# SYSTRAN/faster-whisper

Measured on AMD Instinct MI355X. Metric: audio-sec/sec (RTF) large-v3 fp16 beam=5 batch=16, higher is better.
Workload: dtype f16

## Files before the change

faster_whisper_amd/_lib.py:

```python
import ctypes as C
import os

import numpy as np

_HERE = os.path.dirname(os.path.abspath(__file__))
LIB_PATH = os.environ.get("FWAMD_LIB") or os.path.join(_HERE, "libfwamd.so")

FW_OK = 0
FW_EINVAL = -1
FW_ENODEV = -2
FW_ENOMEM = -3
FW_ERUNTIME = -4
FW_ENOSPC = -5

COMPUTE_FLOAT16 = 0
COMPUTE_INT8_FLOAT16 = 1
FW_DT_F32 = 0
FW_DT_F16 = 1
FW_MAX_ALIGN_HEADS = 64


class FwConfig(C.Structure):
    _fields_ = [
        ("n_mels", C.c_int32), ("n_audio_ctx", C.c_int32), ("d_model", C.c_int32), ("n_heads", C.c_int32),
        ("n_enc_layers", C.c_int32), ("n_dec_layers", C.c_int32), ("n_vocab", C.c_int32),
        ("n_text_ctx", C.c_int32), ("is_multilingual", C.c_int32),
        ("tok_eot", C.c_int32), ("tok_sot", C.c_int32), ("tok_lang_begin", C.c_int32), ("n_langs", C.c_int32),
        ("tok_translate", C.c_int32), ("tok_transcribe", C.c_int32), ("tok_sot_lm", C.c_int32),
        ("tok_sot_prev", C.c_int32), ("tok_no_speech", C.c_int32), ("tok_no_timestamps", C.c_int32),
        ("tok_timestamp_begin", C.c_int32),
        ("n_suppress_begin", C.c_int32), ("suppress_begin", C.c_int32 * 8),
        ("n_align_heads", C.c_int32), ("align_heads", C.c_int32 * (2 * FW_MAX_ALIGN_HEADS)),
    ]


class FwWeight(C.Structure):
    _fields_ = [("name", C.c_char_p), ("data", C.c_void_p), ("dtype", C.c_int32), ("ndim", C.c_int32),
                ("dims", C.c_int64 * 4)]


class FwGenOpts(C.Structure):
    _fields_ = [
        ("beam_size", C.c_int32), ("patience", C.c_float), ("num_hypotheses", C.c_int32),
        ("length_penalty", C.c_float), ("repetition_penalty", C.c_float), ("no_repeat_ngram_size", C.c_int32),
        ("max_length", C.c_int32), ("return_scores", C.c_int32), ("return_no_speech_prob", C.c_int32),
        ("max_initial_timestamp_index", C.c_int32), ("suppress_blank", C.c_int32),
        ("suppress_tokens", C.POINTER(C.c_int32)), ("n_suppress_tokens", C.c_int32),
        ("sampling_topk", C.c_int32), ("sampling_temperature", C.c_float), ("seed", C.c_uint64),
        ("min_new_tokens", C.c_int32),
    ]


class FwVadWeights(C.Structure):
    _fields_ = [
        ("stft_basis", C.c_void_p), ("conv_w", C.c_void_p * 4), ("conv_b", C.c_void_p * 4),
        ("lstm_w", C.c_void_p), ("lstm_r", C.c_void_p), ("lstm_b", C.c_void_p), ("dec_w", C.c_void_p),
        ("dec_b", C.c_float),
    ]


SYMBOLS = [
    "fw_last_error", "fw_abi_version", "fw_device_count",
    "fw_model_create", "fw_model_free", "fw_model_info", "fw_model_blob", "fw_model_create_from_blob_dev",
    "fw_model_set_decode_batch", "fw_model_decode_batch", "fw_model_join_decoder", "fw_model_decode_stats",
    "fw_model_set_merge_wait", "fw_model_set_decode_lanes", "fw_model_run_capacity", "fw_dec_big_min_rows", "fw_dec_big_min_rows_of", "fw_test_knob",
    "fw_test_idle_lead_chunks",
    "fw_pack_blob_size", "fw_pack_blob_copy", "fw_pack_blob_free",
    "fw_logmel", "fw_logmel_full",
    "fw_encode", "fw_encode_pcm", "fw_encode_pcm_dev", "fw_tensor_shape", "fw_tensor_to_host",
    "fw_tensor_from_host", "fw_tensor_free",
    "fw_generate", "fw_detect_language", "fw_align",
    "fw_prof_enable", "fw_prof_reset", "fw_prof_count", "fw_prof_name", "fw_prof_get", "fw_synchronize",
    "fw_dev_alloc", "fw_dev_free", "fw_dev_upload",
    "fw_test_gemm", "fw_test_layernorm", "fw_test_attention", "fw_test_dec_linear", "fw_test_dec_logits", "fw_test_logits_rules",
    "fw_test_dec_self_attn", "fw_test_dec_cross_attn", "fw_test_dec_cross_probs", "fw_test_dec_softmax_pick", "fw_bench_gemm", "fw_bench_dec_linear", "fw_bench_attention",
    "fw_vad_create", "fw_vad_forward", "fw_vad_free", "fw_vad_forward_dev", "fw_vad_forward_audio_dev",
    "fw_flac_info", "fw_flac_decode",
]

_lib = None


class FwError(RuntimeError):
    pass


def load():
    global _lib
    if _lib is not None:
        return _lib
    if not os.path.exists(LIB_PATH):
        raise FwError(
            f"{LIB_PATH} not found: build it with `python -c 'import __graft_entry__ as g; g.build()'` "
            "(hipcc --offload-arch=gfx950). faster_whisper_amd has no CPU fallback.")
    lib = C.CDLL(LIB_PATH)
    vp, i32, i64, f32p = C.c_void_p, C.c_int32, C.c_int64, C.POINTER(C.c_float)
    i32p, i64p = C.POINTER(C.c_int32), C.POINTER(C.c_int64)
    lib.fw_last_error.restype = C.c_char_p
    lib.fw_abi_version.restype = i32
    lib.fw_device_count.restype = i32
    lib.fw_model_create.argtypes = [C.POINTER(FwConfig), C.POINTER(FwWeight), i32, i32, i32, i32, i32, C.POINTER(vp)]
    lib.fw_model_free.argtypes = [vp]
    lib.fw_model_free.restype = None
    lib.fw_model_info.argtypes = [vp, C.POINTER(FwConfig), i32p, i32p, i32p, i32p]
    lib.fw_model_blob.argtypes = [vp, C.POINTER(vp), i64p]
    lib.fw_model_create_from_blob_dev.argtypes = [C.POINTER(FwConfig), vp, i64, i32, i32, i32, i32, C.POINTER(vp)]
    lib.fw_model_set_decode_batch.argtypes = [vp, i32]
    lib.fw_model_decode_batch.argtypes = [vp]
    lib.fw_model_decode_batch.restype = i32
    lib.fw_model_run_capacity.argtypes = [vp]
    lib.fw_model_run_capacity.restype = i32
    lib.fw_dec_big_min_rows.restype = i32
    if hasattr(lib, "fw_dec_big_min_rows_of"):
        lib.fw_dec_big_min_rows_of.restype = i32
        lib.fw_dec_big_min_rows_of.argtypes = [i32, i32]
    if hasattr(lib, "fw_flac_info"):
        lib.fw_flac_info.argtypes = [vp, i64, i32p, i32p, i32p, i64p]
        lib.fw_flac_decode.argtypes = [vp, i64, vp, i64, i64p, i32p]
    if hasattr(lib, "fw_test_knob"):
        lib.fw_test_knob.argtypes = [i32, i32]
    if hasattr(lib, "fw_test_idle_lead_chunks"):
        lib.fw_test_idle_lead_chunks.argtypes = [i64, i32, i32, i64, i32]
        lib.fw_test_idle_lead_chunks.restype = i64
    lib.fw_model_join_decoder.argtypes = [vp, vp]
    lib.fw_model_set_merge_wait.argtypes = [vp, i32, i32]
    lib.fw_model_set_decode_lanes.argtypes = [vp, i32]
    lib.fw_model_decode_stats.argtypes = [vp, i64p, i64p, i64p, i32p]
    lib.fw_pack_blob_size.argtypes = [C.POINTER(FwConfig), C.POINTER(FwWeight), i32, i32, i64p, C.POINTER(vp)]
    lib.fw_pack_blob_copy.argtypes = [vp, vp, i64]
    lib.fw_pack_blob_free.argtypes = [vp]
    lib.fw_pack_blob_free.restype = None
    lib.fw_logmel.argtypes = [vp, vp, i64p, i32, vp, i32p]
    lib.fw_logmel_full.argtypes = [vp, vp, i64, vp, i64]
    lib.fw_encode.argtypes = [vp, vp, i32, C.POINTER(vp)]
    lib.fw_encode_pcm.argtypes = [vp, vp, i64p, i32, C.POINTER(vp)]
    lib.fw_encode_pcm_dev.argtypes = [vp, vp, i64p, i32, C.POINTER(vp)]
    lib.fw_tensor_shape.argtypes = [vp, i32p, i32p, i32p]
    lib.fw_tensor_to_host.argtypes = [vp, vp, vp]
    lib.fw_tensor_from_host.argtypes = [vp, vp, i32, C.POINTER(vp)]
    lib.fw_tensor_free.argtypes = [vp]
    lib.fw_tensor_free.restype = None
    lib.fw_generate.argtypes = [vp, vp, i32p, i32p, i32, C.POINTER(FwGenOpts), i32p, i32p, f32p, f32p]
    lib.fw_detect_language.argtypes = [vp, vp, i32, i32p, f32p]
    lib.fw_align.argtypes = [vp, vp, i32p, i32, i32p, i32p, i32p, i32, i32, i32, i32p, i32p, f32p]
    lib.fw_prof_enable.argtypes = [vp, i32]
    lib.fw_prof_enable.restype = None
    lib.fw_prof_reset.argtypes = [vp]
    lib.fw_prof_reset.restype = None
    lib.fw_prof_count.restype = i32
    lib.fw_prof_name.argtypes = [i32]
    lib.fw_prof_name.restype = C.c_char_p
    lib.fw_prof_get.argtypes = [vp, i32, C.POINTER(C.c_double), i64p, C.POINTER(C.c_double), C.POINTER(C.c_double)]
    lib.fw_synchronize.argtypes = [vp]
    lib.fw_dev_alloc.argtypes = [vp, i64, C.POINTER(vp)]
    lib.fw_dev_free.argtypes = [vp, vp]
    lib.fw_dev_upload.argtypes = [vp, vp, vp, i64]
    lib.fw_test_gemm.argtypes = [vp, vp, vp, vp, vp, i32, i32, i32, i32, i32, vp]
    lib.fw_test_dec_linear.argtypes = [vp, vp, vp, vp, vp, vp, vp, i32, i32, i32, i32, i32, vp, vp]
    lib.fw_test_dec_logits.argtypes = [vp, vp, i32, vp]
    lib.fw_test_logits_rules.argtypes = [vp, vp, i32, vp, i32, vp, C.POINTER(FwGenOpts), i32, vp, vp]
    if hasattr(lib, "fw_test_dec_self_attn"):
        lib.fw_test_dec_self_attn.argtypes = [vp, vp, vp, vp, vp, i32, i32, i32, i32, i32, i32, i32, i32, i32, i32, i32, vp]
        lib.fw_test_dec_cross_attn.argtypes = [vp, vp, vp, vp, i32, i32, i32, i32, i32, i32, vp, vp, i32, C.c_float, vp]
        lib.fw_test_dec_cross_probs.argtypes = [vp, vp, vp, i32, i32, i32, vp, i32, i32, i32, i32, vp]
        lib.fw_test_dec_softmax_pick.argtypes = [vp, vp, i32, i32, i32, vp, i32, vp]
    lib.fw_bench_attention.argtypes = [vp, i32, i32, i32, i32, i32, f32p]
    lib.fw_bench_gemm.argtypes = [vp, i32, i32, i32, i32, i32, i32, i32, i32, f32p]
    lib.fw_bench_dec_linear.argtypes = [vp, i32, i32, i32, i32, i32, i32, f32p]
    lib.fw_test_layernorm.argtypes = [vp, vp, vp, vp, i32, i32, vp]
    lib.fw_test_attention.argtypes = [vp, vp, vp, vp, i32, i32, i32, vp]
    lib.fw_vad_create.argtypes = [C.POINTER(FwVadWeights), C.POINTER(vp)]
    lib.fw_vad_forward.argtypes = [vp, vp, i64, i32, vp, vp, vp]
    lib.fw_vad_free.argtypes = [vp]
    lib.fw_vad_forward_dev.argtypes = [vp, i32, vp, i64, vp, vp, vp]
    if hasattr(lib, "fw_vad_forward_audio_dev"):
        lib.fw_vad_forward_audio_dev.argtypes = [vp, i32, vp, i64, vp, vp, vp]
    lib.fw_vad_free.restype = None
    _lib = lib
    return lib


def check(rc: int):
    if rc == FW_OK:
        return
    msg = load().fw_last_error().decode("utf-8", "replace")
    if rc in (FW_EINVAL, FW_ENOSPC):
        raise ValueError(msg)
    raise RuntimeError(f"libfwamd error {rc}: {msg}")


def ptr(a: np.ndarray):
    return a.ctypes.data_as(C.c_void_p)


def as_i32p(a: np.ndarray):
    return a.ctypes.data_as(C.POINTER(C.c_int32))


def as_i64p(a: np.ndarray):
    return a.ctypes.data_as(C.POINTER(C.c_int64))


def as_f32p(a: np.ndarray):
    return a.ctypes.data_as(C.POINTER(C.c_float))
```

faster_whisper_amd/csrc/dec_kernels.hip:

```cpp
#include "common.h"
#include "dec_kernels.h"
#include <stdlib.h>
#include <atomic>
#include <type_traits>

namespace fwd {
static std::atomic<int> g_self_attn_form{0};
static std::atomic<int> g_forms_epoch{0};
static std::atomic<int> g_cross_regs{0};
}

__device__ __forceinline__ size_t frag_off(int row, int k, int KS) {
  return ((size_t)((row >> 4) * KS + (k >> 5)) * 64 + ((k >> 3) & 3) * 16 + (row & 15)) * 8 + (k & 7);
}

__global__ void dec_embed_kernel(const int* __restrict__ tok, const half_t* __restrict__ emb,
                                 const half_t* __restrict__ pos_emb, half_t* __restrict__ x,
                                 half_t* __restrict__ xfrag, int d, const int* __restrict__ d_step, int pos_fixed,
                                 int P, int blk_n) {
  const int r = blockIdx.x;
  const int pos = blk_n > 0 ? pos_fixed + r % blk_n : (pos_fixed >= 0 ? pos_fixed : P - 1 + *d_step);
  const half2_t* e = reinterpret_cast<const half2_t*>(emb + (size_t)tok[r] * d);
  const half2_t* pe = reinterpret_cast<const half2_t*>(pos_emb + (size_t)pos * d);
  half2_t* xo = reinterpret_cast<half2_t*>(x + (size_t)r * d);
  for (int i = threadIdx.x; i < d / 2; i += blockDim.x) {
    const half2_t a = e[i], b = pe[i];
    half2_t o;
    o[0] = (half_t)((float)a[0] + (float)b[0]);
    o[1] = (half_t)((float)a[1] + (float)b[1]);
    xo[i] = o;
    if (xfrag) *reinterpret_cast<half2_t*>(xfrag + frag_off(r, 2 * i, d >> 5)) = o;
  }
}

static __device__ __forceinline__ void dec_ln_stats(float sa, float sb, int K, float& mu, float& rstd) {
#pragma clang fp contract(off)
  const float kf = (float)K;
  mu = sa / kf;
  const float ex2 = sb / kf;
  const float var = ex2 - mu * mu;
  rstd = rsqrtf(fmaxf(var, 0.f) + 1e-5f);
}
template <bool LNF>
static __device__ __forceinline__ half4_t dec_epilogue4(const floatx4 v, float mu, float rstd,
                                                        const float* __restrict__ s1, const float* __restrict__ cf,
                                                        const half_t* __restrict__ bias, bool has_res, half4_t r4, int n, int act) {
#pragma clang fp contract(off)
  floatx4 a4 = {0.f, 0.f, 0.f, 0.f}, c4 = {0.f, 0.f, 0.f, 0.f};
  half4_t b4 = {(half_t)0.f, (half_t)0.f, (half_t)0.f, (half_t)0.f};
  if (LNF) {
    a4 = *reinterpret_cast<const floatx4*>(s1 + n);
    c4 = *reinterpret_cast<const floatx4*>(cf + n);
  } else if (bias) {
    b4 = *reinterpret_cast<const half4_t*>(bias + n);
  }
  half4_t o;
#pragma unroll
  for (int e = 0; e < 4; ++e) {
    float tv = v[e];
    if (LNF) {
      const float t = tv - mu * a4[e];
      tv = rstd * t + c4[e];
    } else if (bias) {
      tv = tv + (float)b4[e];
    }
    if (act == 1) {
      const float er = erff(tv * 0.70710678118654752440f);
      tv = (0.5f * tv) * (1.0f + er);
    }
    if (has_res) tv = tv + (float)r4[e];
    o[e] = (half_t)tv;
  }
  return o;
}

static __device__ __forceinline__ half4_t dec_epilogue4_i8(const int (&v)[4], float sx, const float* __restrict__ w_scale,
                                                           const half_t* __restrict__ bias, const half_t* __restrict__ res,
                                                           int ldr, int row, int n, int act) {
#pragma clang fp contract(off)
  const floatx4 w4 = *reinterpret_cast<const floatx4*>(w_scale + n);
  half4_t b4 = {(half_t)0.f, (half_t)0.f, (half_t)0.f, (half_t)0.f}, r4 = b4;
  if (bias) b4 = *reinterpret_cast<const half4_t*>(bias + n);
  if (res) r4 = *reinterpret_cast<const half4_t*>(res + (size_t)row * ldr + n);
  half4_t o;
#pragma unroll
  for (int e = 0; e < 4; ++e) {
    float tv = ((float)v[e] * sx) * w4[e];
    if (bias) tv = tv + (float)b4[e];
    if (act == 1) {
      const float er = erff(tv * 0.70710678118654752440f);
      tv = (0.5f * tv) * (1.0f + er);
    }
    if (res) tv = tv + (float)r4[e];
    o[e] = (half_t)tv;
  }
  return o;
}

template <int WAVES, bool LNF, int RT, int NT, int CH_ = 0>
__global__ __launch_bounds__(WAVES * 64) void dec_gemm_frag_kernel(
    const half_t* __restrict__ xf, const half_t* __restrict__ Wf, const half_t* __restrict__ bias,
    const float* __restrict__ s1, const float* __restrict__ cf, const half_t* __restrict__ res, int ldr,
    half_t* __restrict__ out, int ldo, half_t* __restrict__ out_frag, int R, int N, int K, int act) {
  __shared__ float red[WAVES][RT * NT][64][4];
  __shared__ float red_s[WAVES][RT][16][2];
  constexpr int CH = CH_ ? CH_ : 20 / (RT + NT);
  const int lane = threadIdx.x & 63;
  const int wave = __builtin_amdgcn_readfirstlane(threadIdx.x >> 6);
  const int i = lane & 15, g = lane >> 4;
  const int n_rt = (R + 15) >> 4;
  const int ct0 = blockIdx.x * NT, rt0 = blockIdx.y * RT;
  const int KS = K >> 5;
  const int per = (KS + WAVES - 1) / WAVES;
  const int ks0 = wave * per;
  int nks = KS - ks0;
  if (nks > per) nks = per;
  floatx4 acc[RT][NT];
  float rs[RT], rq[RT];
#pragma unroll
  for (int a = 0; a < RT; ++a) {
    rs[a] = 0.f; rq[a] = 0.f;
#pragma unroll
    for (int b = 0; b < NT; ++b) acc[a][b] = floatx4{0, 0, 0, 0};
  }
  half4_t resv[(RT * NT + WAVES - 1) / WAVES];
#pragma unroll
  for (int q = 0; q < (RT * NT + WAVES - 1) / WAVES; ++q) resv[q] = half4_t{(half_t)0.f, (half_t)0.f, (half_t)0.f, (half_t)0.f};
  if (res) {
#pragma unroll
    for (int a = 0; a < RT; ++a) {
#pragma unroll
      for (int b = 0; b < NT; ++b) {
        if ((a * NT + b) % WAVES != wave) continue;
        const int row = (rt0 + a) * 16 + i, n = (ct0 + b) * 16 + 4 * g;
        if (row < R && n < N) resv[(a * NT + b) / WAVES] = *reinterpret_cast<const half4_t*>(res + (size_t)row * ldr + n);
      }
    }
  }
  if (nks > 0) {
    const half8_t* wp[NT];
    const half8_t* xp[RT];
#pragma unroll
    for (int b = 0; b < NT; ++b) {
      int ct = ct0 + b;
      if (ct > (N >> 4) - 1) ct = (N >> 4) - 1;
      wp[b] = reinterpret_cast<const half8_t*>(Wf) + ((size_t)ct * KS + ks0) * 64 + lane;
    }
#pragma unroll
    for (int a = 0; a < RT; ++a) {
      int rt = rt0 + a;
      if (rt > n_rt - 1) rt = n_rt - 1;
      xp[a] = reinterpret_cast<const half8_t*>(xf) + ((size_t)rt * KS + ks0) * 64 + lane;
    }
    for (int c = 0; c < nks; c += CH) {
      half8_t wv[NT][CH], xv[RT][CH];
#pragma unroll
      for (int j = 0; j < CH; ++j) {
        const int jj = (c + j < nks) ? c + j : nks - 1;
#pragma unroll
        for (int b = 0; b < NT; ++b) wv[b][j] = wp[b][(size_t)jj * 64];
#pragma unroll
        for (int a = 0; a < RT; ++a) xv[a][j] = xp[a][(size_t)jj * 64];
      }
#pragma unroll
      for (int j = 0; j < CH; ++j) {
        if (c + j < nks) {
#pragma unroll
          for (int a = 0; a < RT; ++a) {
#pragma unroll
            for (int b = 0; b < NT; ++b)
              acc[a][b] = __builtin_amdgcn_mfma_f32_16x16x32_f16(wv[b][j], xv[a][j], acc[a][b], 0, 0, 0);
            if (LNF) {
              const half2_t one2 = {(half_t)1.f, (half_t)1.f};
#pragma unroll
              for (int e = 0; e < 4; ++e) {
                const half2_t h2 = {xv[a][j][2 * e], xv[a][j][2 * e + 1]};
                rs[a] = __builtin_amdgcn_fdot2(h2, one2, rs[a], false);
                rq[a] = __builtin_amdgcn_fdot2(h2, h2, rq[a], false);
              }
            }
          }
        }
      }
    }
  }
#pragma unroll
  for (int a = 0; a < RT; ++a) {
    if (LNF) {
      float sa = rs[a], sb = rq[a];
      sa += __shfl_xor(sa, 16, 64); sa += __shfl_xor(sa, 32, 64);
      sb += __shfl_xor(sb, 16, 64); sb += __shfl_xor(sb, 32, 64);
      if (g == 0) { red_s[wave][a][i][0] = sa; red_s[wave][a][i][1] = sb; }
    }
#pragma unroll
    for (int b = 0; b < NT; ++b)
#pragma unroll
      for (int e = 0; e < 4; ++e) red[wave][a * NT + b][lane][e] = acc[a][b][e];
  }
  __syncthreads();
#pragma unroll
  for (int a = 0; a < RT; ++a) {
#pragma unroll
    for (int b = 0; b < NT; ++b) {
      if ((a * NT + b) % WAVES != wave) continue;
      const int row = (rt0 + a) * 16 + i;
      if (row >= R) continue;
      float v[4] = {0.f, 0.f, 0.f, 0.f};
#pragma unroll
      for (int w = 0; w < WAVES; ++w)
#pragma unroll
        for (int e = 0; e < 4; ++e) v[e] += red[w][a * NT + b][lane][e];
      float mu = 0.f, rstd = 1.f;
      if (LNF) {
        float sa = 0.f, sb = 0.f;
#pragma unroll
        for (int w = 0; w < WAVES; ++w) { sa += red_s[w][a][i][0]; sb += red_s[w][a][i][1]; }
        dec_ln_stats(sa, sb, K, mu, rstd);
      }
      const int n = (ct0 + b) * 16 + 4 * g;
      if (n >= N) continue;
      const floatx4 v4 = {v[0], v[1], v[2], v[3]};
      const half4_t r4 = resv[(a * NT + b) / WAVES];
      const half4_t o = dec_epilogue4<LNF>(v4, mu, rstd, s1, cf, bias, res != nullptr, r4, n, act);
      if (out) *reinterpret_cast<half4_t*>(out + (size_t)row * ldo + n) = o;
      if (out_frag) *reinterpret_cast<half4_t*>(out_frag + frag_off(row, n, N >> 5)) = o;
    }
  }
}

#ifndef DGB_TL
#define DGB_TL(slot) do {} while (0)
#define DGB_TL_DECL
#endif
template <int N_>
static __device__ __forceinline__ void wait_vmcnt() {
  asm volatile("s_waitcnt vmcnt(%0)" ::"n"(N_) : "memory");
}
#define DGB_BARRIER()                      \
  do {                                     \
    asm volatile("" ::: "memory");         \
    __builtin_amdgcn_s_barrier();          \
    asm volatile("" ::: "memory");         \
  } while (0)

#define DGB_BARRIER_LDS() __syncthreads()

template <bool LNF, int S, int WM, int WN, int FB, int KC, int NST>
__global__ __launch_bounds__(WM * WN * 64, 2) void dec_gemm_big_kernel(
    const half_t* __restrict__ xf, const half_t* __restrict__ Wf, const half_t* __restrict__ bias,
    const float* __restrict__ s1, const float* __restrict__ cf, const half_t* __restrict__ res, int ldr,
    half_t* __restrict__ out, int ldo, half_t* __restrict__ out_frag, int R, int N, int K, int act, int nNt) {
  constexpr int NW = WM * WN;
  DGB_TL_DECL;
  constexpr int PX = 4 * WM, PW = FB * WN, PCS = PX + PW;
  static_assert((PCS * KC) % NW == 0, "pieces of a stage must divide over the waves");
  static_assert(FB == 2 || FB == 4, "column tiles per wave");
  constexpr int PPW = PCS * KC / NW;
  constexpr int STAGE_BYTES = PCS * KC * 1024;
  static_assert(NST >= 3 && NST <= 6, "ring depth");
  constexpr int DGB_EP_STRIDE = FB * 32 + 16;
  static_assert(NST * STAGE_BYTES >= NW * 64 * DGB_EP_STRIDE, "the epilogue stages one 64-row patch per wave through the ring");
  extern __shared__ __attribute__((aligned(16))) char dgb_smem[];
  const int lane = threadIdx.x & 63;
  const int wave = __builtin_amdgcn_readfirstlane(threadIdx.x >> 6);
  const int i = lane & 15, g = lane >> 4;
  const int wm = wave / WN, wn = wave % WN;
  const int bid = xcd_remap(blockIdx.x, gridDim.x);
  const int nMt = gridDim.x / nNt;
  const int nt = bid / nMt, mt = bid - nt * nMt;
  const int rt0 = mt * PX, ct0 = nt * PW;
  const int n_rt = (R + 15) >> 4;
  const int KS = K >> 5;
  const int per = KS / S;
  const int nch = KS / KC;
  const int ch_per_slice = per / KC;

  unsigned soff[PPW];
  const char* sbase[PPW];
#pragma unroll
  for (int q = 0; q < PPW; ++q) {
    const int p = wave * PPW + q;
    const int t = p / KC, ks = p % KC;
    if (t < PX) {
      int rt = rt0 + t;
      if (rt > n_rt - 1) rt = n_rt - 1;
      sbase[q] = reinterpret_cast<const char*>(xf);
      soff[q] = (unsigned)((((size_t)rt * KS + ks) * 64 + lane) * 16);
    } else {
      int ct = ct0 + t - PX;
      if (ct > (N >> 4) - 1) ct = (N >> 4) - 1;
      sbase[q] = reinterpret_cast<const char*>(Wf);
      soff[q] = (unsigned)((((size_t)ct * KS + ks) * 64 + lane) * 16);
    }
  }
  auto issue = [&](int c, int slot) {
    char* dst = dgb_smem + slot * STAGE_BYTES + wave * PPW * 1024;
    const unsigned koff = (unsigned)c * (KC * 1024);
#pragma unroll
    for (int q = 0; q < PPW; ++q)
      __builtin_amdgcn_global_load_lds((const __attribute__((address_space(1))) void*)(sbase[q] + (size_t)(soff[q] + koff)),
                                       (__attribute__((address_space(3))) void*)(dst + q * 1024), 16, 0, 0);
  };

  static_assert(!LNF || WN == 2, "the LayerNorm statistics are shared by the TWO waves of a row block");
  floatx4 acc[4][FB], tot[4][FB];
  float rs[2] = {0.f, 0.f}, rq[2] = {0.f, 0.f}, sal[2] = {0.f, 0.f}, sbl[2] = {0.f, 0.f};
  float sa[4], sb[4];
#pragma unroll
  for (int a = 0; a < 4; ++a) {
    sa[a] = 0.f; sb[a] = 0.f;
#pragma unroll
    for (int b = 0; b < FB; ++b) { acc[a][b] = floatx4{0, 0, 0, 0}; tot[a][b] = floatx4{0, 0, 0, 0}; }
  }

  half8_t xv[KC][4], wv[KC][FB];
  auto fetch = [&](int slot) {
    const char* st = dgb_smem + slot * STAGE_BYTES;
#pragma unroll
    for (int ks = 0; ks < KC; ++ks) {
#pragma unroll
      for (int a = 0; a < 4; ++a)
        xv[ks][a] = *reinterpret_cast<const half8_t*>(st + (((wm * 4 + a) * KC + ks) * 64 + lane) * 16);
#pragma unroll
      for (int b = 0; b < FB; ++b)
        wv[ks][b] = *reinterpret_cast<const half8_t*>(st + (((PX + wn * FB + b) * KC + ks) * 64 + lane) * 16);
    }
    __builtin_amdgcn_sched_barrier(0);
  };
  auto mma = [&]() {
    __builtin_amdgcn_sched_barrier(0);
    DGB_TL(4);
#pragma unroll
    for (int ks = 0; ks < KC; ++ks) {
      if (LNF) {
        const half2_t one2 = {(half_t)1.f, (half_t)1.f};
        const half8_t xs0 = wn ? xv[ks][2] : xv[ks][0], xs1 = wn ? xv[ks][3] : xv[ks][1];
#pragma unroll
        for (int e = 0; e < 4; ++e) {
          const half2_t h0 = {xs0[2 * e], xs0[2 * e + 1]}, h1 = {xs1[2 * e], xs1[2 * e + 1]};
          rs[0] = __builtin_amdgcn_fdot2(h0, one2, rs[0], false);
          rq[0] = __builtin_amdgcn_fdot2(h0, h0, rq[0], false);
          rs[1] = __builtin_amdgcn_fdot2(h1, one2, rs[1], false);
          rq[1] = __builtin_amdgcn_fdot2(h1, h1, rq[1], false);
        }
      }
#pragma unroll
      for (int b = 0; b < FB; ++b) {
#pragma unroll
        for (int a = 0; a < 4; ++a)
          acc[a][b] = __builtin_amdgcn_mfma_f32_16x16x32_f16(wv[ks][b], xv[ks][a], acc[a][b], 0, 0, 0);
      }
    }
  };
  auto compute = [&](int slot) { fetch(slot); mma(); };
  auto slice_end = [&]() {
    if (LNF) {
#pragma unroll
      for (int aa = 0; aa < 2; ++aa) {
        float pa = rs[aa], pb = rq[aa];
        pa += __shfl_xor(pa, 16, 64); pa += __shfl_xor(pa, 32, 64);
        pb += __shfl_xor(pb, 16, 64); pb += __shfl_xor(pb, 32, 64);
        sal[aa] += pa; sbl[aa] += pb;
        rs[aa] = 0.f; rq[aa] = 0.f;
      }
    }
#pragma unroll
    for (int a = 0; a < 4; ++a) {
#pragma unroll
      for (int b = 0; b < FB; ++b) {
#pragma unroll
        for (int e = 0; e < 4; ++e) tot[a][b][e] += acc[a][b][e];
        acc[a][b] = floatx4{0, 0, 0, 0};
      }
    }
  };

#pragma unroll
  for (int c0 = 0; c0 < NST - 1; ++c0) issue(c0, c0);
  int slot = 0, fill = NST - 1;
  int to_slice = ch_per_slice;
  const int n_steady = nch - (NST - 1);
  for (int c = 0; c < n_steady; ++c) {
    DGB_TL(0);
    wait_vmcnt<(NST - 2) * PPW>();
    DGB_TL(1);
    DGB_BARRIER();
    DGB_TL(2);
    fetch(slot);
    DGB_TL(3);
    issue(c + NST - 1, fill);
    mma();
    DGB_TL(5);
    if (--to_slice == 0) { to_slice = ch_per_slice; slice_end(); }
    fill = slot;
    slot = (slot + 1 == NST) ? 0 : slot + 1;
  }
  wait_vmcnt<0>();
#pragma unroll 1
  for (int c = n_steady; c < nch; ++c) {
    DGB_BARRIER();
    compute(slot);
    if (--to_slice == 0) { to_slice = ch_per_slice; slice_end(); }
    slot = (slot + 1 == NST) ? 0 : slot + 1;
  }
  DGB_BARRIER();

  if (LNF) {
    float* xch = reinterpret_cast<float*>(dgb_smem);
    if (g == 0) {
#pragma unroll
      for (int aa = 0; aa < 2; ++aa) {
        xch[((wave * 2 + aa) * 16 + i) * 2] = sal[aa];
        xch[((wave * 2 + aa) * 16 + i) * 2 + 1] = sbl[aa];
      }
    }
    DGB_BARRIER_LDS();
#pragma unroll
    for (int a = 0; a < 4; ++a) {
      const int owner = (wave & ~1) | (a >> 1);
      sa[a] = xch[((owner * 2 + (a & 1)) * 16 + i) * 2];
      sb[a] = xch[((owner * 2 + (a & 1)) * 16 + i) * 2 + 1];
    }
    DGB_BARRIER_LDS();
  }
  char* ep = dgb_smem + wave * (64 * DGB_EP_STRIDE);
  const int row0 = (rt0 + wm * 4) * 16;
  const int col0 = (ct0 + wn * FB) * 16;
  constexpr int CPR = FB * 2;
  constexpr int RPI = 64 / CPR;
  const int cr = lane / CPR, cc = lane % CPR;
  if (res) {
#pragma unroll
    for (int j = 0; j < 64 / RPI; ++j) {
      const int r = j * RPI + cr;
      const int row = row0 + r, n = col0 + cc * 8;
      intx4 v = {0, 0, 0, 0};
      if (row < R && n < N) v = *reinterpret_cast<const intx4*>(res + (size_t)row * ldr + n);
      *reinterpret_cast<intx4*>(ep + r * DGB_EP_STRIDE + cc * 16) = v;
    }
  }
#pragma unroll
  for (int a = 0; a < 4; ++a) {
    float mu = 0.f, rstd = 1.f;
    if (LNF) dec_ln_stats(sa[a], sb[a], K, mu, rstd);
#pragma unroll
    for (int b = 0; b < FB; ++b) {
      int n = col0 + b * 16 + 4 * g;
      if (n > N - 4) n = N - 4;
      char* cell = ep + (a * 16 + i) * DGB_EP_STRIDE + (b * 16 + 4 * g) * 2;
      half4_t r4 = {(half_t)0.f, (half_t)0.f, (half_t)0.f, (half_t)0.f};
      if (res) r4 = *reinterpret_cast<const half4_t*>(cell);
      const half4_t o = dec_epilogue4<LNF>(tot[a][b], mu, rstd, s1, cf, bias, res != nullptr, r4, n, act);
      *reinterpret_cast<half4_t*>(cell) = o;
    }
  }
  if (out) {
#pragma unroll
    for (int j = 0; j < 64 / RPI; ++j) {
      const int r = j * RPI + cr;
      const int row = row0 + r, n = col0 + cc * 8;
      const intx4 v = *reinterpret_cast<const intx4*>(ep + r * DGB_EP_STRIDE + cc * 16);
      if (row < R && n < N) *reinterpret_cast<intx4*>(out + (size_t)row * ldo + n) = v;
    }
  }
  if (out_frag) {
    const int KSo = N >> 5;
#pragma unroll
    for (int a = 0; a < 4; ++a) {
#pragma unroll
      for (int kb = 0; kb < FB / 2; ++kb) {
        const int row = row0 + a * 16 + i, n = col0 + kb * 32 + g * 8;
        const intx4 v = *reinterpret_cast<const intx4*>(ep + (a * 16 + i) * DGB_EP_STRIDE + (kb * 32 + g * 8) * 2);
        if (row < R && n < N)
          *reinterpret_cast<intx4*>(out_frag + ((size_t)((row >> 4) * KSo + (n >> 5)) * 64 + lane) * 8) = v;
      }
    }
  }
}

template <int WAVES, int RT, int NT, int CH_ = 0>
__global__ __launch_bounds__(WAVES * 64) void dec_gemm_frag_i8_kernel(
    const int8_t* __restrict__ xq, const float* __restrict__ x_scale, const int8_t* __restrict__ Wq,
    const float* __restrict__ w_scale, const half_t* __restrict__ bias, const half_t* __restrict__ res, int ldr,
    half_t* __restrict__ out, int ldo, int R, int N, int K, int act) {
  __shared__ int red[WAVES][RT * NT][64][4];
  constexpr int CH = CH_ ? CH_ : 20 / (RT + NT);
  const int lane = threadIdx.x & 63;
  const int wave = __builtin_amdgcn_readfirstlane(threadIdx.x >> 6);
  const int i = lane & 15, g = lane >> 4;
  const int ct0 = blockIdx.x * NT, rt0 = blockIdx.y * RT;
  const int n_rt = (R + 15) >> 4;
  const int KS = K >> 6;
  const int per = (KS + WAVES - 1) / WAVES;
  const int ks0 = wave * per;
  int nks = KS - ks0;
  if (nks > per) nks = per;
  intx4 acc[RT][NT];
#pragma unroll
  for (int a = 0; a < RT; ++a)
#pragma unroll
    for (int b = 0; b < NT; ++b) acc[a][b] = intx4{0, 0, 0, 0};
  if (nks > 0) {
    const intx4* wp[NT];
    const intx4* xp[RT];
#pragma unroll
    for (int b = 0; b < NT; ++b)
      wp[b] = reinterpret_cast<const intx4*>(Wq) + ((size_t)(ct0 + b) * KS + ks0) * 64 + lane;
#pragma unroll
    for (int a = 0; a < RT; ++a) {
      int rt = rt0 + a;
      if (rt > n_rt - 1) rt = n_rt - 1;
      xp[a] = reinterpret_cast<const intx4*>(xq) + ((size_t)rt * KS + ks0) * 64 + lane;
    }
    for (int c = 0; c < nks; c += CH) {
      intx4 wv[NT][CH], xv[RT][CH];
#pragma unroll
      for (int j = 0; j < CH; ++j) {
        const int jj = (c + j < nks) ? c + j : nks - 1;
#pragma unroll
        for (int b = 0; b < NT; ++b) wv[b][j] = wp[b][(size_t)jj * 64];
#pragma unroll
        for (int a = 0; a < RT; ++a) xv[a][j] = xp[a][(size_t)jj * 64];
      }
#pragma unroll
      for (int j = 0; j < CH; ++j) {
        if (c + j < nks) {
#pragma unroll
          for (int a = 0; a < RT; ++a)
#pragma unroll
            for (int b = 0; b < NT; ++b)
              acc[a][b] = __builtin_amdgcn_mfma_i32_16x16x64_i8(wv[b][j], xv[a][j], acc[a][b], 0, 0, 0);
        }
      }
    }
  }
#pragma unroll
  for (int a = 0; a < RT; ++a)
#pragma unroll
    for (int b = 0; b < NT; ++b)
#pragma unroll
      for (int e = 0; e < 4; ++e) red[wave][a * NT + b][lane][e] = acc[a][b][e];
  __syncthreads();
#pragma unroll
  for (int a = 0; a < RT; ++a) {
#pragma unroll
    for (int b = 0; b < NT; ++b) {
      if ((a * NT + b) % WAVES != wave) continue;
      const int row = (rt0 + a) * 16 + i;
      if (row >= R) continue;
      int v[4] = {0, 0, 0, 0};
#pragma unroll
      for (int w = 0; w < WAVES; ++w)
#pragma unroll
        for (int e = 0; e < 4; ++e) v[e] += red[w][a * NT + b][lane][e];
      const float sx = x_scale[row];
      const int n = (ct0 + b) * 16 + 4 * g;
      const half4_t o = dec_epilogue4_i8(v, sx, w_scale, bias, res, ldr, row, n, act);
      *reinterpret_cast<half4_t*>(out + (size_t)row * ldo + n) = o;
    }
  }
}

template <bool I8, bool LNF, bool F32, int RT, int NT, int WM, int WN>
__global__ __launch_bounds__(WM * WN * 64) void dec_gemm_wave_kernel(
    const void* __restrict__ xfv, const float* __restrict__ x_scale, const void* __restrict__ Wfv,
    const float* __restrict__ w_scale, const half_t* __restrict__ bias, const float* __restrict__ s1,
    const float* __restrict__ cf, void* __restrict__ outv, int ldo, int R, int N, int K, int n_rg) {
  constexpr int CH = 2;
  const int lane = threadIdx.x & 63;
  const int wave = __builtin_amdgcn_readfirstlane(threadIdx.x >> 6);
  const int wm = wave / WN, wn = wave - wm * WN;
  const int i = lane & 15, g = lane >> 4;
  const int n_rt = (R + 15) >> 4, n_ct = (N + 15) >> 4;
  const int b8 = blockIdx.x >> 3;
  const int cgrp = (b8 / n_rg) * 8 + (blockIdx.x & 7), rgrp = b8 % n_rg;
  const int rt0 = (rgrp * WM + wm) * RT, ct0 = (cgrp * WN + wn) * NT;
  constexpr bool SPLIT = LNF && WM == 1 && WN == 4 && RT >= 4;
  __shared__ float xst[SPLIT ? RT : 1][16][2];
  if (rt0 >= n_rt) return;
  if (!SPLIT && ct0 >= n_ct) return;
  const int KS = K / (I8 ? 64 : 32);
  const intx4* wp[NT];
  const intx4* xp[RT];
#pragma unroll
  for (int b = 0; b < NT; ++b) {
    int ct = ct0 + b; if (ct > n_ct - 1) ct = n_ct - 1;
    wp[b] = reinterpret_cast<const intx4*>(Wfv) + (size_t)ct * KS * 64 + lane;
  }
#pragma unroll
  for (int a = 0; a < RT; ++a) {
    int rt = rt0 + a; if (rt > n_rt - 1) rt = n_rt - 1;
    xp[a] = reinterpret_cast<const intx4*>(xfv) + (size_t)rt * KS * 64 + lane;
  }
  floatx4 accf[RT][NT];
  intx4 acci[RT][NT];
  float rs[RT], rq[RT];
#pragma unroll
  for (int a = 0; a < RT; ++a) {
    rs[a] = 0.f; rq[a] = 0.f;
#pragma unroll
    for (int b = 0; b < NT; ++b) { accf[a][b] = floatx4{0, 0, 0, 0}; acci[a][b] = intx4{0, 0, 0, 0}; }
  }
  struct Set { intx4 w[CH][NT]; intx4 x[CH][RT]; };
  auto load = [&](Set& f, int ks0) {
#pragma unroll
    for (int j = 0; j < CH; ++j) {
      int ks = ks0 + j; if (ks > KS - 1) ks = KS - 1;
#pragma unroll
      for (int b = 0; b < NT; ++b) f.w[j][b] = wp[b][(size_t)ks * 64];
#pragma unroll
      for (int a = 0; a < RT; ++a) f.x[j][a] = xp[a][(size_t)ks * 64];
    }
  };
  auto compute = [&](const Set& f, int ks0) {
#pragma unroll
    for (int j = 0; j < CH; ++j) {
      if (ks0 + j < KS) {
#pragma unroll
        for (int a = 0; a < RT; ++a) {
#pragma unroll
          for (int b = 0; b < NT; ++b) {
            if (I8) acci[a][b] = __builtin_amdgcn_mfma_i32_16x16x64_i8(f.w[j][b], f.x[j][a], acci[a][b], 0, 0, 0);
            else accf[a][b] = __builtin_amdgcn_mfma_f32_16x16x32_f16(__builtin_bit_cast(half8_t, f.w[j][b]),
                                                                    __builtin_bit_cast(half8_t, f.x[j][a]), accf[a][b],
                                                                    0, 0, 0);
          }
          if (LNF && !SPLIT) {
            const half8_t xv = __builtin_bit_cast(half8_t, f.x[j][a]);
            const half2_t one2 = {(half_t)1.f, (half_t)1.f};
#pragma unroll
            for (int e = 0; e < 4; ++e) {
              const half2_t h2 = {xv[2 * e], xv[2 * e + 1]};
              rs[a] = __builtin_amdgcn_fdot2(h2, one2, rs[a], false);
              rq[a] = __builtin_amdgcn_fdot2(h2, h2, rq[a], false);
            }
          }
        }
        if (SPLIT) {
          const half2_t one2 = {(half_t)1.f, (half_t)1.f};
          const intx4 xsel = wn == 0 ? f.x[j][0] : (wn == 1 ? f.x[j][1] : (wn == 2 ? f.x[j][2] : f.x[j][RT > 3 ? 3 : 0]));
          const half8_t xv = __builtin_bit_cast(half8_t, xsel);
#pragma unroll
          for (int e = 0; e < 4; ++e) {
            const half2_t h2 = {xv[2 * e], xv[2 * e + 1]};
            rs[0] = __builtin_amdgcn_fdot2(h2, one2, rs[0], false);
            rq[0] = __builtin_amdgcn_fdot2(h2, h2, rq[0], false);
          }
          if (RT > 4 && wn == 0) {
            const half8_t xw = __builtin_bit_cast(half8_t, f.x[j][RT > 4 ? 4 : 0]);
#pragma unroll
            for (int e = 0; e < 4; ++e) {
              const half2_t h2 = {xw[2 * e], xw[2 * e + 1]};
              rs[1] = __builtin_amdgcn_fdot2(h2, one2, rs[1], false);
              rq[1] = __builtin_amdgcn_fdot2(h2, h2, rq[1], false);
            }
          }
        }
      }
    }
  };
  Set fa, fb;
  load(fa, 0);
  for (int ks0 = 0; ks0 < KS; ks0 += 2 * CH) {
    load(fb, ks0 + CH);
    compute(fa, ks0);
    load(fa, ks0 + 2 * CH);
    compute(fb, ks0 + CH);
  }
  if (SPLIT) {
#pragma unroll
    for (int q = 0; q < 2; ++q) {
      if (q == 1 && !(RT > 4 && wn == 0)) break;
      float sa = rs[q], sb = rq[q];
      sa += __shfl_xor(sa, 16, 64); sa += __shfl_xor(sa, 32, 64);
      sb += __shfl_xor(sb, 16, 64); sb += __shfl_xor(sb, 32, 64);
      if (g == 0) { xst[q == 0 ? wn : 4][i][0] = sa; xst[q == 0 ? wn : 4][i][1] = sb; }
    }
    __syncthreads();
  }
#pragma unroll
  for (int a = 0; a < RT; ++a) {
    float mu = 0.f, rstd = 1.f;
    if (LNF) {
      float sa, sb;
      if (SPLIT) {
        sa = xst[a][i][0]; sb = xst[a][i][1];
      } else {
        sa = rs[a]; sb = rq[a];
        sa += __shfl_xor(sa, 16, 64); sa += __shfl_xor(sa, 32, 64);
        sb += __shfl_xor(sb, 16, 64); sb += __shfl_xor(sb, 32, 64);
      }
      mu = sa / (float)K;
      rstd = rsqrtf(fmaxf(sb / (float)K - mu * mu, 0.f) + 1e-5f);
    }
    const int row = (rt0 + a) * 16 + i;
    if (rt0 + a >= n_rt || row >= R) continue;
    const float sx = I8 ? x_scale[row] : 1.f;
    const bool pair_ok = (ldo & 1) == 0;
#pragma unroll
    for (int b = 0; b < NT; ++b) {
      if (ct0 + b >= n_ct) continue;
      const int n = (ct0 + b) * 16 + 4 * g;
      float t4[4];
#pragma unroll
      for (int e = 0; e < 4; ++e) {
        const int ne = n + e < N ? n + e : N - 1;
        float tv = I8 ? (float)acci[a][b][e] * sx * w_scale[ne] : accf[a][b][e];
        if (LNF) tv = rstd * (tv - mu * s1[ne]) + cf[ne];
        else if (bias) tv += (float)bias[ne];
        t4[e] = tv;
      }
      if (F32 && pair_ok) {
        float* o = reinterpret_cast<float*>(outv) + (size_t)row * ldo + n;
        if (n + 1 < N) *reinterpret_cast<floatx2*>(o) = floatx2{t4[0], t4[1]};
        else if (n < N) o[0] = t4[0];
        if (n + 3 < N) *reinterpret_cast<floatx2*>(o + 2) = floatx2{t4[2], t4[3]};
        else if (n + 2 < N) o[2] = t4[2];
        continue;
      }
#pragma unroll
      for (int e = 0; e < 4; ++e) {
        if (n + e >= N) continue;
        if (F32) reinterpret_cast<float*>(outv)[(size_t)row * ldo + n + e] = t4[e];
        else reinterpret_cast<half_t*>(outv)[(size_t)row * ldo + n + e] = (half_t)t4[e];
      }
    }
  }
}

#define SA_MAX_CTX 448
static __device__ __forceinline__ float sum8_dpp(float v) {
  v += __builtin_bit_cast(float, __builtin_amdgcn_update_dpp(0, __builtin_bit_cast(int, v), 0xB1, 0xF, 0xF, true));
  v += __builtin_bit_cast(float, __builtin_amdgcn_update_dpp(0, __builtin_bit_cast(int, v), 0x4E, 0xF, 0xF, true));
  v += __builtin_bit_cast(float, __builtin_amdgcn_update_dpp(0, __builtin_bit_cast(int, v), 0x141, 0xF, 0xF, true));
  return v;
}
__global__ __launch_bounds__(1024) __attribute__((amdgpu_waves_per_eu(8, 8))) void dec_self_attn_kernel(const half_t* __restrict__ qkv, int d, half_t* __restrict__ kc,
                                                             half_t* __restrict__ vc, int n_ctx, int cache_ctx,
                                                             int H, const uint8_t* __restrict__ kvidx2, int Kbeam, int kmul,
                                                             half_t* __restrict__ out, const int* __restrict__ d_step,
                                                             int pos_fixed, int P, int R_total, int frag) {
  extern __shared__ float sa_smem[];
  const int lane = threadIdx.x & 63;
  const int wave = __builtin_amdgcn_readfirstlane(threadIdx.x >> 6);
  float* sp = sa_smem + (size_t)wave * 2 * n_ctx;
  int* ssrc = reinterpret_cast<int*>(sp + n_ctx);
  const int h = blockIdx.x, c = blockIdx.y;
  const int r = c * kmul + wave, kb = wave;
  const int step = *d_step;
  const int pos = pos_fixed >= 0 ? pos_fixed : P - 1 + step;
  const int slot = c * Kbeam + kb;
  const int cur = (pos_fixed >= 0) ? 0 : (step & 1);
  const uint8_t* kvidx = kvidx2 + ((size_t)cur * R_total + slot) * n_ctx;
  const half_t* qr = qkv + (size_t)r * 3 * d + h * 64;
  const size_t head_stride = (size_t)cache_ctx * 64;
  const size_t slot_stride = (size_t)H * head_stride;
  const int pg = lane >> 3, cc = lane & 7;
  const half8_t q8 = *reinterpret_cast<const half8_t*>(qr + cc * 8);
  const half8_t kn8 = *reinterpret_cast<const half8_t*>(qr + d + cc * 8);
  const half8_t vn8 = *reinterpret_cast<const half8_t*>(qr + 2 * d + cc * 8);
  float q[8];
#pragma unroll
  for (int e = 0; e < 8; ++e) q[e] = (float)q8[e] * 0.125f;
  if (pg == 0) {
    *reinterpret_cast<half8_t*>(kc + slot * slot_stride + h * head_stride + (size_t)pos * 64 + cc * 8) = kn8;
    *reinterpret_cast<half8_t*>(vc + slot * slot_stride + h * head_stride + (size_t)pos * 64 + cc * 8) = vn8;
  }
  auto dot8 = [&](const half8_t& k) {
    float sacc = 0.f;
#pragma unroll
    for (int e = 0; e < 8; ++e) sacc += q[e] * (float)k[e];
    return sum8_dpp(sacc);
  };
  const float s_new = dot8(kn8);
  float mx = s_new;
  const half_t* kbase = kc + h * head_stride + cc * 8;
  for (int p0 = 0; p0 < pos; p0 += 32) {
    half8_t kv[4];
    int src[4];
#pragma unroll
    for (int j = 0; j < 4; ++j) {
      const int p = p0 + 8 * j + pg;
      const int pc = p < pos ? p : pos - 1;
      src[j] = c * Kbeam + kvidx[pc];
      kv[j] = *reinterpret_cast<const half8_t*>(kbase + src[j] * slot_stride + (size_t)pc * 64);
    }
#pragma unroll
    for (int j = 0; j < 4; ++j) {
      const int p = p0 + 8 * j + pg;
      const float sc = dot8(kv[j]);
      if (p < pos) {
        if (cc == 0) { sp[p] = sc; ssrc[p] = src[j]; }
        mx = fmaxf(mx, sc);
      }
    }
  }
  mx = wave_max(mx);
  __builtin_amdgcn_wave_barrier();
  float sum = 0.f;
  for (int p = lane; p < pos; p += 64) {
    const float e = __expf(sp[p] - mx);
    sp[p] = e;
    sum += e;
  }
  const float e_new = __expf(s_new - mx);
  sum = wave_sum(sum) + e_new;
  __builtin_amdgcn_wave_barrier();
  float acc[8];
#pragma unroll
  for (int e = 0; e < 8; ++e) acc[e] = 0.f;
  const half_t* vb = vc + h * head_stride + cc * 8;
#pragma unroll 4
  for (int p = pg; p < pos; p += 8) {
    const half8_t vv = *reinterpret_cast<const half8_t*>(vb + ssrc[p] * slot_stride + (size_t)p * 64);
    const float w = sp[p];
#pragma unroll
    for (int e = 0; e < 8; ++e) acc[e] += w * (float)vv[e];
  }
#pragma unroll
  for (int e = 0; e < 8; ++e) {
    float a = acc[e];
    a += __shfl_xor(a, 8, 64);
    a += __shfl_xor(a, 16, 64);
    a += __shfl_xor(a, 32, 64);
    acc[e] = a;
  }
  if (pg == 0) {
    const float inv = 1.f / sum;
    half8_t o;
#pragma unroll
    for (int e = 0; e < 8; ++e) o[e] = (half_t)((acc[e] + e_new * (float)vn8[e]) * inv);
    half_t* dst = frag ? out + frag_off(r, h * 64 + cc * 8, d >> 5) : out + (size_t)r * d + h * 64 + cc * 8;
    *reinterpret_cast<half8_t*>(dst) = o;
  }
}

template <int U, bool PIPE, int MAXT, bool PB = false>
__global__ __launch_bounds__(MAXT) void dec_self_attn2_kernel(const half_t* __restrict__ qkv, int d, half_t* __restrict__ kc,
                                                             half_t* __restrict__ vc, int n_ctx, int cache_ctx,
                                                             int H, const uint8_t* __restrict__ kvidx2, int Kbeam, int kmul,
                                                             half_t* __restrict__ out, const int* __restrict__ d_step,
                                                             int pos_fixed, int P, int R_total, int frag) {
  extern __shared__ float sa_smem[];
  constexpr int NB = 4 * U;
  const int lane = threadIdx.x & 63;
  const int wave = __builtin_amdgcn_readfirstlane(threadIdx.x >> 6);
  float* sp = sa_smem + (size_t)wave * 2 * n_ctx;
  int* ssrc = reinterpret_cast<int*>(sp + n_ctx);
  const int h = blockIdx.x, c = blockIdx.y;
  const int r = c * kmul + wave, kb = PB ? 0 : wave;
  const int step = PB ? 0 : *d_step;
  const int pos = PB ? pos_fixed + wave : (pos_fixed >= 0 ? pos_fixed : P - 1 + step);
  const int slot = c * Kbeam + kb;
  const int cur = (pos_fixed >= 0) ? 0 : (step & 1);
  const uint8_t* kvidx = kvidx2 + ((size_t)cur * R_total + slot) * n_ctx;
  const half_t* qr = qkv + (size_t)r * 3 * d + h * 64;
  const size_t head_stride = (size_t)cache_ctx * 64;
  const size_t slot_stride = (size_t)H * head_stride;
  const int pg = lane >> 3, cc = lane & 7;
  for (int p4 = 4 * lane; p4 < pos; p4 += 256) {
    const unsigned w = PB ? 0u : *reinterpret_cast<const unsigned*>(kvidx + p4);
    intx4 s4;
    s4[0] = c * Kbeam + (int)(w & 0xffu); s4[1] = c * Kbeam + (int)((w >> 8) & 0xffu);
    s4[2] = c * Kbeam + (int)((w >> 16) & 0xffu); s4[3] = c * Kbeam + (int)(w >> 24);
    *reinterpret_cast<intx4*>(ssrc + p4) = s4;
  }
  const half8_t q8 = *reinterpret_cast<const half8_t*>(qr + cc * 8);
  const half8_t kn8 = *reinterpret_cast<const half8_t*>(qr + d + cc * 8);
  const half8_t vn8 = *reinterpret_cast<const half8_t*>(qr + 2 * d + cc * 8);
  float q[8];
#pragma unroll
  for (int e = 0; e < 8; ++e) q[e] = (float)q8[e] * 0.125f;
  if (pg == 0) {
    *reinterpret_cast<half8_t*>(kc + slot * slot_stride + h * head_stride + (size_t)pos * 64 + cc * 8) = kn8;
    *reinterpret_cast<half8_t*>(vc + slot * slot_stride + h * head_stride + (size_t)pos * 64 + cc * 8) = vn8;
  }
  auto dot8 = [&](const half8_t& k) {
    float sacc = 0.f;
#pragma unroll
    for (int e = 0; e < 8; ++e) sacc = __builtin_fmaf(q[e], (float)k[e], sacc);
    return sum8_dpp(sacc);
  };
  const float s_new = dot8(kn8);
  float mx = s_new;
  __builtin_amdgcn_wave_barrier();
  const char* kbase = reinterpret_cast<const char*>(kc + h * head_stride);
  const char* vbase = reinterpret_cast<const char*>(vc + h * head_stride);
  const unsigned slot_bytes = (unsigned)(slot_stride * sizeof(half_t));
  struct Batch { half8_t row[NB]; };
  auto fetch = [&](Batch& b, const char* base, int p0, const half_t* sib) {
#pragma unroll
    for (int j = 0; j < NB; ++j) {
      const int p = p0 + 8 * j + pg;
      const int pc = p < pos ? p : pos - 1;
      const unsigned off = (unsigned)ssrc[pc] * slot_bytes + (unsigned)(pc * 128 + cc * 16);
      if (PB && pc >= pos_fixed)
        b.row[j] = *reinterpret_cast<const half8_t*>(sib + (size_t)(pc - pos_fixed) * 3 * d + cc * 8);
      else
        b.row[j] = *reinterpret_cast<const half8_t*>(base + off);
    }
  };
  const half_t* ksib = qkv + (size_t)c * kmul * 3 * d + d + h * 64;
  const half_t* vsib = ksib + d;
  auto score = [&](const Batch& b, int p0) {
#pragma unroll
    for (int j = 0; j < NB; ++j) {
      const int p = p0 + 8 * j + pg;
      const float sc = dot8(b.row[j]);
      if (p < pos) {
        if (cc == 0) sp[p] = sc;
        mx = fmaxf(mx, sc);
      }
    }
  };
  Batch b0, b1;
  if (pos > 0) {
    fetch(b0, kbase, 0, ksib);
    for (int p0 = 0; p0 < pos; p0 += 16 * NB) {
      if (PIPE) {
        fetch(b1, kbase, p0 + 8 * NB, ksib);
        score(b0, p0);
        fetch(b0, kbase, p0 + 16 * NB, ksib);
        score(b1, p0 + 8 * NB);
      } else {
        score(b0, p0);
        if (p0 + 8 * NB < pos) {
          fetch(b0, kbase, p0 + 8 * NB, ksib);
          score(b0, p0 + 8 * NB);
          if (p0 + 16 * NB < pos) fetch(b0, kbase, p0 + 16 * NB, ksib);
        }
      }
    }
    fetch(b0, vbase, 0, vsib);
  }
  mx = wave_max_v(mx);
  __builtin_amdgcn_wave_barrier();
  float sum = 0.f;
  for (int p = lane; p < pos; p += 64) {
    const float e = __expf(sp[p] - mx);
    sp[p] = e;
    sum += e;
  }
  const float e_new = __expf(s_new - mx);
  sum = wave_sum_v(sum) + e_new;
  __builtin_amdgcn_wave_barrier();
  float acc[8];
#pragma unroll
  for (int e = 0; e < 8; ++e) acc[e] = 0.f;
  auto accum = [&](const Batch& b, int p0) {
#pragma unroll
    for (int j = 0; j < NB; ++j) {
      const int p = p0 + 8 * j + pg;
      if (p < pos) {
        const float w = sp[p];
#pragma unroll
        for (int e = 0; e < 8; ++e) acc[e] = __builtin_fmaf(w, (float)b.row[j][e], acc[e]);
      }
    }
  };
  for (int p0 = 0; p0 < pos; p0 += 16 * NB) {
    if (PIPE) {
      fetch(b1, vbase, p0 + 8 * NB, vsib);
      accum(b0, p0);
      fetch(b0, vbase, p0 + 16 * NB, vsib);
      accum(b1, p0 + 8 * NB);
    } else {
      accum(b0, p0);
      if (p0 + 8 * NB < pos) {
        fetch(b0, vbase, p0 + 8 * NB, vsib);
        accum(b0, p0 + 8 * NB);
        if (p0 + 16 * NB < pos) fetch(b0, vbase, p0 + 16 * NB, vsib);
      }
    }
  }
#pragma unroll
  for (int e = 0; e < 8; ++e) acc[e] = sum_x8_x16_x32_v(acc[e]);
  if (pg == 0) {
    const float inv = 1.f / sum;
    half8_t o;
#pragma unroll
    for (int e = 0; e < 8; ++e) o[e] = (half_t)((acc[e] + e_new * (float)vn8[e]) * inv);
    half_t* dst = frag ? out + frag_off(r, h * 64 + cc * 8, d >> 5) : out + (size_t)r * d + h * 64 + cc * 8;
    *reinterpret_cast<half8_t*>(dst) = o;
  }
}

template <int CA_WAVES, bool NTL, int MINW = 1>
__global__ __launch_bounds__(CA_WAVES * 64, MINW) void dec_cross_attn_kernel(const half_t* __restrict__ qx, int d,
                                                             const half_t* __restrict__ ck,
                                                             const half_t* __restrict__ cvt, int T, int kvp,
                                                             int kmul, half_t* __restrict__ out,
                                                             const int* __restrict__ done, int kv_div, int frag,
                                                             const int* __restrict__ slot_map) {
  __shared__ float sm[CA_WAVES][16], sl[CA_WAVES][16];
  __shared__ float so[CA_WAVES][16][65];
  const int h = blockIdx.x, c = blockIdx.y;
  if (done && done[c]) return;
  const int tid = threadIdx.x, lane = tid & 63, wave = tid >> 6;
  const int j = lane & 15, g = lane >> 4;
  const int ce = slot_map[c / kv_div];
  const half_t* kbase = ck + ((size_t)ce * (d >> 6) + h) * kvp * 64 + lane * 8;
  const half_t* vbase = cvt + ((size_t)ce * (d >> 6) + h) * kvp * 64 + lane * 8;
  half8_t qf[2];
  {
    if (j < kmul) {
      const half_t* qp = qx + (size_t)(c * kmul + j) * d + h * 64 + g * 8;
#pragma unroll
      for (int s = 0; s < 2; ++s) {
        half8_t v = *reinterpret_cast<const half8_t*>(qp + s * 32);
#pragma unroll
        for (int e = 0; e < 8; ++e) v[e] = v[e] * (half_t)0.125f;
        qf[s] = v;
// ... 815 lines not shown
```

faster_whisper_amd/csrc/engine.hip:

```cpp
#include "engine.h"

#include <math.h>
#include <stdarg.h>
#include <stdio.h>
#include <stdlib.h>
#include <string.h>

#include <algorithm>

#include "dec_kernels.h"
#include "kernels.h"

namespace fw {

static thread_local char g_err[1024] = "";
void set_error(const char* fmt, ...) {
  va_list ap;
  va_start(ap, fmt);
  vsnprintf(g_err, sizeof(g_err), fmt, ap);
  va_end(ap);
}

int dev_alloc(void** p, size_t bytes) {
  if (bytes == 0) bytes = 256;
// ... 1662 lines not shown

static inline size_t frag_pos(int64_t row, int64_t k, int64_t K, int KE) {
  const int OCT = KE / 4;
  return (size_t)((((row >> 4) * (K / KE) + k / KE) * 64 + ((k / OCT) & 3) * 16 + (row & 15)) * OCT + (k % OCT));
}

int32_t fw_test_dec_linear(fw_model* fm, const float* x, const float* W, const float* bias, const float* ln_g,
                           const float* ln_b, const float* res, int32_t R, int32_t N, int32_t K, int32_t act,
                           int32_t use_int8, float* out, float* out_from_frag) {
  FW_CHECK_ARG(fm && x && W && out && out_from_frag, "null argument");
  FW_CHECK_ARG(R >= 1 && N % 32 == 0 && K % 64 == 0, "need R >= 1, N %% 32 == 0, K %% 64 == 0");
  FW_CHECK_ARG((ln_g == nullptr) == (ln_b == nullptr), "ln_g and ln_b go together");
  Model* m = &fm->impl;
  std::lock_guard<std::mutex> lk(m->mu);
  FW_HIP(hipSetDevice(m->device));
  hipStream_t st = m->stream;
  const int R16 = (R + 15) / 16 * 16;
  auto h = [](float v) { return f16_bits_to_f32(f32_to_f16_bits(v)); };
  std::vector<void*> owned;
  auto up = [&](const void* src, size_t bytes, void** dst) -> int {
    int rc = dev_alloc(dst, bytes);
    if (rc) return rc;
    owned.push_back(*dst);
    FW_HIP(hipMemcpy(*dst, src, bytes, hipMemcpyHostToDevice));
    return FW_OK;
  };
  auto cleanup = [&]() { for (void* p : owned) (void)hipFree(p); };
  int rc = FW_OK;
  half_t *d_res = nullptr, *d_bias = nullptr, *d_out = nullptr, *d_of = nullptr;
  std::vector<uint16_t> tmp;
  if (res) {
    tmp.resize((size_t)R * N);
    for (size_t i = 0; i < tmp.size(); ++i) tmp[i] = f32_to_f16_bits(res[i]);
    if ((rc = up(tmp.data(), tmp.size() * 2, (void**)&d_res))) { cleanup(); return rc; }
  }
  if ((rc = dev_alloc_t(&d_out, (size_t)R * N))) { cleanup(); return rc; }
  owned.push_back(d_out);
  if ((rc = dev_alloc_t(&d_of, (size_t)R16 * N))) { cleanup(); return rc; }
  owned.push_back(d_of);
  FW_HIP(hipMemset(d_of, 0, (size_t)R16 * N * 2));
  if (use_int8 == 1) {
    if (m->compute_type != FW_COMPUTE_INT8_FLOAT16 || ln_g) {
      cleanup();
      set_error("int8 decoder-linear test needs an int8_float16 model and no LayerNorm");
      return FW_EINVAL;
    }
    std::vector<int8_t> wq((size_t)N * K);
    std::vector<float> ws(N);
    for (int n = 0; n < N; ++n) {
      float amax = 0.f;
      for (int k = 0; k < K; ++k) amax = std::max(amax, fabsf(h(W[(size_t)n * K + k])));
      const float sc = amax > 0.f ? 127.0f / amax : 0.f;
      for (int k = 0; k < K; ++k) wq[frag_pos(n, k, K, 64)] = (int8_t)lrintf(h(W[(size_t)n * K + k]) * sc);
      ws[n] = amax > 0.f ? amax / 127.0f : 1.0f;
    }
    int8_t *d_wq = nullptr, *d_xq = nullptr;
    float *d_ws = nullptr, *d_xs = nullptr;
    half_t* d_x = nullptr;
    tmp.resize((size_t)R * K);
    for (size_t i = 0; i < tmp.size(); ++i) tmp[i] = f32_to_f16_bits(x[i]);
    if ((rc = up(wq.data(), wq.size(), (void**)&d_wq)) || (rc = up(ws.data(), ws.size() * 4, (void**)&d_ws)) ||
        (rc = up(tmp.data(), tmp.size() * 2, (void**)&d_x))) { cleanup(); return rc; }
    if (bias) {
      tmp.resize(N);
      for (int n = 0; n < N; ++n) tmp[n] = f32_to_f16_bits(bias[n]);
      if ((rc = up(tmp.data(), (size_t)N * 2, (void**)&d_bias))) { cleanup(); return rc; }
    }
    if ((rc = dev_alloc_t(&d_xq, (size_t)R16 * K))) { cleanup(); return rc; }
    owned.push_back(d_xq);
    if ((rc = dev_alloc_t(&d_xs, (size_t)R16))) { cleanup(); return rc; }
    owned.push_back(d_xs);
    FW_HIP(hipMemset(d_xq, 0, (size_t)R16 * K));
    fwk::launch_quant_rows(st, d_x, K, nullptr, nullptr, d_xq, d_xs, R, K, 1);
    if (fwd::launch_dec_gemm_frag_i8(st, d_xq, d_xs, d_wq, d_ws, d_bias, d_res, N, d_out, N, R, N, K, act) != 0) {
      cleanup();
      set_error("int8 decoder linear: unsupported shape R=%d N=%d K=%d", R, N, K);
      return FW_ERUNTIME;
    }
    rc = download_f16(m, d_out, (size_t)R * N, out);
    if (!rc) memcpy(out_from_frag, out, (size_t)R * N * sizeof(float));
    cleanup();
    return rc;
  }
  std::vector<uint16_t> wf((size_t)N * K), xf((size_t)R16 * K, 0);
  std::vector<float> s1(N, 0.f), cf(N, 0.f);
  for (int n = 0; n < N; ++n) {
    double a1 = 0.0, ac = 0.0;
    for (int k = 0; k < K; ++k) {
      const float wv = h(W[(size_t)n * K + k]);
      const uint16_t wg = ln_g ? f32_to_f16_bits(wv * h(ln_g[k])) : f32_to_f16_bits(wv);
      wf[frag_pos(n, k, K, 32)] = wg;
      a1 += (double)f16_bits_to_f32(wg);
      if (ln_g) ac += (double)wv * (double)h(ln_b[k]);
    }
    if (bias) ac += (double)h(bias[n]);
    s1[n] = (float)a1;
    cf[n] = (float)ac;
  }
  for (int r = 0; r < R; ++r)
    for (int k = 0; k < K; ++k) xf[frag_pos(r, k, K, 32)] = f32_to_f16_bits(x[(size_t)r * K + k]);
  half_t *d_wf = nullptr, *d_xf = nullptr;
  float *d_s1 = nullptr, *d_cf = nullptr;
  if ((rc = up(wf.data(), wf.size() * 2, (void**)&d_wf)) || (rc = up(xf.data(), xf.size() * 2, (void**)&d_xf))) {
    cleanup();
    return rc;
  }
  if (ln_g) {
    if ((rc = up(s1.data(), (size_t)N * 4, (void**)&d_s1)) || (rc = up(cf.data(), (size_t)N * 4, (void**)&d_cf))) {
      cleanup();
      return rc;
    }
  } else if (bias) {
    tmp.resize(N);
    for (int n = 0; n < N; ++n) tmp[n] = f32_to_f16_bits(bias[n]);
    if ((rc = up(tmp.data(), (size_t)N * 2, (void**)&d_bias))) { cleanup(); return rc; }
  }
  const int lr =
      use_int8 >= 10 ? fwd::launch_dec_gemm_big(st, use_int8 - 10, d_xf, d_wf, d_bias, d_s1, d_cf, d_res, N, d_out, N, d_of, R, N, K, act)
      : use_int8 == 5 ? fwd::launch_dec_gemm_skinny(st, d_xf, d_wf, d_bias, d_s1, d_cf, d_res, N, d_out, N, d_of, R, N, K, act)
      : (use_int8 == 6 || use_int8 == 7) ? fwd::launch_dec_gemm_skinny_tiles(st, use_int8 - 5, d_xf, d_wf, d_bias, d_s1, d_cf, d_res, N, d_out, N, d_of, R, N, K, act)
                      : fwd::launch_dec_gemm_frag(st, d_xf, d_wf, d_bias, d_s1, d_cf, d_res, N, d_out, N, d_of, R, N, K, act);
  if (lr != 0) {
    cleanup();
    set_error("decoder linear: unsupported shape R=%d N=%d K=%d", R, N, K);
    return FW_ERUNTIME;
  }
  rc = download_f16(m, d_out, (size_t)R * N, out);
  std::vector<float> of((size_t)R16 * N);
  if (!rc) rc = download_f16(m, d_of, (size_t)R16 * N, of.data());
  if (!rc)
    for (int r = 0; r < R; ++r)
      for (int n = 0; n < N; ++n) out_from_frag[(size_t)r * N + n] = of[frag_pos(r, n, N, 32)];
  cleanup();
  return rc;
}

int32_t fw_dec_big_min_rows(void) { return fwd::dec_big_min_rows(); }
int32_t fw_dec_big_min_rows_of(int32_t role, int32_t compute_type) { return fwd::dec_big_min_rows_of(role, compute_type); }

int32_t fw_test_knob(int32_t id, int32_t value) {
  FW_CHECK_ARG(id == 1 || id == 2 || id == 4 || id == 5 || id == 6 || id == 7, "unknown knob %d", id);
  if (id == 6) { set_cross_kv_layered(value); return FW_OK; }
  if (id == 7) { fwd::set_cross_attn_regs(value); return FW_OK; }
  if (id == 1) fwk::g_gemm_order.store(value);
  else if (id == 5) fwk::g_gemm_vt_stage.store(value);
  else if (id == 2) fwd::set_self_attn_form(value);
  else set_pos_blocks(value);
  return FW_OK;
}

int64_t fw_test_idle_lead_chunks(int64_t queued, int32_t n_queued, int32_t encoding, int64_t want, int32_t max_batch) {
  return idle_lead_chunks(queued, n_queued, encoding, want, max_batch);
}

int32_t fw_test_dec_logits(fw_model* fm, const float* x, int32_t R, float* out) {
  FW_CHECK_ARG(fm && x && out && R >= 1, "bad argument");
  Model* m = &fm->impl;
  std::lock_guard<std::mutex> lk(m->mu);
  FW_HIP(hipSetDevice(m->device));
  hipStream_t st = m->stream;
  const int d = m->cfg.d_model, V = m->cfg.n_vocab, R16 = (R + 15) / 16 * 16;
  const bool i8 = m->compute_type == FW_COMPUTE_INT8_FLOAT16;
  std::vector<uint16_t> xh((size_t)R16 * d, 0);
  for (int r = 0; r < R; ++r)
    for (int k = 0; k < d; ++k)
      xh[i8 ? (size_t)r * d + k : frag_pos(r, k, d, 32)] = f32_to_f16_bits(x[(size_t)r * d + k]);
  half_t* d_x = nullptr;
  int8_t* d_xq = nullptr;
  float *d_xs = nullptr, *d_out = nullptr;
  int rc;
  auto cleanup = [&]() { for (void* p : {(void*)d_x, (void*)d_xq, (void*)d_xs, (void*)d_out}) if (p) (void)hipFree(p); };
  if ((rc = dev_alloc_t(&d_x, xh.size())) || (rc = dev_alloc_t(&d_out, (size_t)R * V))) { cleanup(); return rc; }
  FW_HIP(hipMemcpy(d_x, xh.data(), xh.size() * 2, hipMemcpyHostToDevice));
  int lr;
  if (i8) {
    if ((rc = dev_alloc_t(&d_xq, (size_t)R16 * d)) || (rc = dev_alloc_t(&d_xs, (size_t)R16))) { cleanup(); return rc; }
    FW_HIP(hipMemset(d_xq, 0, (size_t)R16 * d));
    fwk::launch_quant_rows(st, d_x, d, m->dec_ln.g, m->dec_ln.b, d_xq, d_xs, R, d, 1);
    lr = fwd::launch_dec_logits(st, true, d_xq, d_xs, m->logits.wq, m->logits.wscale, nullptr, nullptr, d_out, V, R, V, d);
  } else {
    lr = fwd::launch_dec_logits(st, false, d_x, nullptr, m->logits.w, nullptr, m->logits.s1, m->logits.cf, d_out, V, R, V,
                                d);
  }
  hipError_t he = hipSuccess;
  if (lr == 0) he = hipMemcpyAsync(out, d_out, (size_t)R * V * sizeof(float), hipMemcpyDeviceToHost, st);
  if (he == hipSuccess) he = hipStreamSynchronize(st);
  cleanup();
  if (lr != 0 || he != hipSuccess) {
    set_error("logits projection test failed: %s", lr ? "unsupported shape" : hipGetErrorString(he));
    return FW_ERUNTIME;
  }
  return FW_OK;
}

int32_t fw_bench_dec_linear(fw_model* fm, int32_t R, int32_t N, int32_t K, int32_t lnf, int32_t variant, int32_t iters,
                            float* us_out) {
  FW_CHECK_ARG(fm && us_out && R > 0 && N > 0 && K > 0 && iters > 0, "bad argument");
  Model* m = &fm->impl;
  std::lock_guard<std::mutex> lk(m->mu);
  FW_HIP(hipSetDevice(m->device));
  const size_t wn = (size_t)N * K;
  const int copies = (int)std::max<size_t>(2, ((size_t)640 << 20) / (wn * 2));
  const size_t rp = ((size_t)R + 15) / 16 * 16;
  half_t *dW = nullptr, *dX = nullptr, *dO = nullptr, *dB = nullptr;
  float *dS = nullptr, *dC = nullptr;
  int rc;
  auto cleanup = [&]() { for (void* p : {(void*)dW, (void*)dX, (void*)dO, (void*)dB, (void*)dS, (void*)dC}) if (p) (void)hipFree(p); };
  if ((rc = dev_alloc_t(&dW, wn * copies)) || (rc = dev_alloc_t(&dX, rp * K)) || (rc = dev_alloc_t(&dO, rp * N)) ||
      (rc = dev_alloc_t(&dB, (size_t)N)) || (rc = dev_alloc_t(&dS, (size_t)N)) || (rc = dev_alloc_t(&dC, (size_t)N))) {
    cleanup();
    return rc;
  }
  {
    std::vector<uint16_t> h(std::max(wn, rp * (size_t)K));
    uint32_t sd = 2463534242u;
    for (auto& v : h) { sd = sd * 1664525u + 1013904223u; v = f32_to_f16_bits(((int)(sd >> 16) % 2001 - 1000) * 1e-3f); }
    for (int c = 0; c < copies; ++c) FW_HIP(hipMemcpy(dW + (size_t)c * wn, h.data(), wn * 2, hipMemcpyHostToDevice));
    FW_HIP(hipMemcpy(dX, h.data(), rp * K * 2, hipMemcpyHostToDevice));
  }
  FW_HIP(hipMemset(dB, 0, (size_t)N * 2));
  FW_HIP(hipMemset(dS, 0, (size_t)N * 4));
  FW_HIP(hipMemset(dC, 0, (size_t)N * 4));
  hipEvent_t e0, e1;
  FW_HIP(hipEventCreate(&e0));
  FW_HIP(hipEventCreate(&e1));
  hipStream_t st = m->stream;
  int lr = 0;
  for (int i = 0; i < 4 && lr == 0; ++i)
    lr = fwd::launch_dec_gemm_frag_variant(st, variant, lnf != 0, dX, dW + (size_t)(i % copies) * wn, dB, dS, dC, dO, R, N, K);
  FW_HIP(hipEventRecord(e0, st));
  for (int i = 0; i < iters && lr == 0; ++i)
    lr = fwd::launch_dec_gemm_frag_variant(st, variant, lnf != 0, dX, dW + (size_t)(i % copies) * wn, dB, dS, dC, dO, R, N, K);
  FW_HIP(hipEventRecord(e1, st));
  hipError_t he = hipEventSynchronize(e1);
  float ms = 0.f;
  if (he == hipSuccess) he = hipEventElapsedTime(&ms, e0, e1);
  (void)hipEventDestroy(e0);
  (void)hipEventDestroy(e1);
  cleanup();
  if (lr != 0) { set_error("fw_bench_dec_linear: unsupported shape / variant"); return FW_EINVAL; }
  if (he != hipSuccess) { set_error("fw_bench_dec_linear: %s", hipGetErrorString(he)); return FW_ENODEV; }
  *us_out = ms * 1000.f / (float)iters;
  return FW_OK;
}

int32_t fw_bench_gemm(fw_model* fm, int32_t M, int32_t N, int32_t K, int32_t batch, int32_t a_pad, int32_t w_pad,
                      int32_t trans, int32_t iters, float* ms_out) {
  FW_CHECK_ARG(fm && ms_out && M > 0 && N > 0 && K > 0 && batch > 0 && iters > 0, "bad argument");
  Model* m = &fm->impl;
  std::lock_guard<std::mutex> lk(m->mu);
  FW_HIP(hipSetDevice(m->device));
  const bool i8 = m->compute_type == FW_COMPUTE_INT8_FLOAT16;
  const int64_t lda = K + a_pad, ldw = K + w_pad;
  const size_t es = i8 ? 1 : 2;
  const int64_t ldct = (M + 63) / 64 * 64;
  const size_t na = (size_t)batch * M * lda, nw = (size_t)N * ldw,
               nc = trans ? (size_t)batch * N * ldct : (size_t)batch * M * N;
  void *dA = nullptr, *dW = nullptr;
  half_t* dC = nullptr;
  float *dsa = nullptr, *dsw = nullptr;
  int rc;
  auto cleanup = [&]() { for (void* p : {dA, dW, (void*)dC, (void*)dsa, (void*)dsw}) if (p) (void)hipFree(p); };
  if ((rc = dev_alloc(&dA, na * es)) || (rc = dev_alloc(&dW, nw * es)) || (rc = dev_alloc_t(&dC, nc))) { cleanup(); return rc; }
  {
    std::vector<uint16_t> h(std::max(na, nw));
    uint32_t st = 12345u;
    for (auto& v : h) { st = st * 1664525u + 1013904223u; v = f32_to_f16_bits(((int)(st >> 16) % 2001 - 1000) * 1e-3f); }
    FW_HIP(hipMemcpy(dA, h.data(), na * es, hipMemcpyHostToDevice));
    FW_HIP(hipMemcpy(dW, h.data(), nw * es, hipMemcpyHostToDevice));
  }
  if (i8) {
    if ((rc = dev_alloc_t(&dsa, (size_t)batch * M)) || (rc = dev_alloc_t(&dsw, (size_t)N))) { cleanup(); return rc; }
    FW_HIP(hipMemset(dsa, 0, (size_t)batch * M * 4));
    FW_HIP(hipMemset(dsw, 0, (size_t)N * 4));
  }
  fwk::GemmParams p;
  memset(&p, 0, sizeof(p));
  p.A = (const half_t*)dA; p.lda = lda; p.a_bstride = (int64_t)M * lda;
  p.W = (const half_t*)dW; p.ldw = ldw;
  p.C = dC; p.ldc = trans ? ldct : N; p.c_bstride = trans ? (int64_t)N * ldct : (int64_t)M * N;
  p.M = M; p.N = N; p.K = K;
  p.a_scale = dsa; p.as_bstride = M; p.w_scale = dsw;
  hipEvent_t e0, e1;
  FW_HIP(hipEventCreate(&e0));
  FW_HIP(hipEventCreate(&e1));
  int lr = fwk::launch_gemm(m->stream, p, batch, trans != 0);
  FW_HIP(hipEventRecord(e0, m->stream));
  for (int i = 0; i < iters && lr == 0; ++i) lr = fwk::launch_gemm(m->stream, p, batch, trans != 0);
  FW_HIP(hipEventRecord(e1, m->stream));
  hipError_t he = hipEventSynchronize(e1);
  float ms = 0.f;
  if (he == hipSuccess) he = hipEventElapsedTime(&ms, e0, e1);
  (void)hipEventDestroy(e0);
  (void)hipEventDestroy(e1);
  cleanup();
  if (lr != 0 || he != hipSuccess) {
    set_error("gemm bench failed: %s", lr ? "unsupported shape" : hipGetErrorString(he));
    return FW_ERUNTIME;
  }
  *ms_out = ms / (float)iters;
  return FW_OK;
}

int32_t fw_test_layernorm(fw_model* fm, const float* x, const float* g, const float* b, int32_t rows, int32_t d,
                          float* out) {
  FW_CHECK_ARG(fm && x && g && b && out, "null argument");
  FW_CHECK_ARG(d % 128 == 0 && d <= 1280, "d must be a multiple of 128 and <= 1280");
  Model* m = &fm->impl;
  std::lock_guard<std::mutex> lk(m->mu);
  FW_HIP(hipSetDevice(m->device));
  half_t *dx = nullptr, *dg = nullptr, *db = nullptr, *dy = nullptr;
  int rc;
  if ((rc = upload_f16(m, x, (size_t)rows * d, &dx))) return rc;
  if ((rc = upload_f16(m, g, d, &dg))) return rc;
  if ((rc = upload_f16(m, b, d, &db))) return rc;
  if ((rc = dev_alloc_t(&dy, (size_t)rows * d))) return rc;
  fwk::launch_layernorm(m->stream, dx, dg, db, dy, rows, d);
  rc = download_f16(m, dy, (size_t)rows * d, out);
  for (half_t* p : {dx, dg, db, dy})
    if (p) (void)hipFree(p);
  return rc;
}

int32_t fw_test_attention(fw_model* fm, const float* q, const float* k, const float* v, int32_t B, int32_t H,
                          int32_t T, float* out) {
  FW_CHECK_ARG(fm && q && k && v && out, "null argument");
  Model* m = &fm->impl;
  std::lock_guard<std::mutex> lk(m->mu);
  FW_HIP(hipSetDevice(m->device));
  const int d = H * 64, tp = (T + 63) / 64 * 64;
  const size_t n = (size_t)B * T * d;
  half_t *dq = nullptr, *dk = nullptr, *dvt = nullptr, *dout = nullptr;
  int rc;
  if ((rc = upload_f16(m, q, n, &dq))) return rc;
  if ((rc = upload_f16(m, k, n, &dk))) return rc;
  std::vector<float> vt((size_t)B * d * tp, 0.f);
  for (int b = 0; b < B; ++b)
    for (int t = 0; t < T; ++t)
      for (int c = 0; c < d; ++c) vt[((size_t)b * d + c) * tp + t] = v[((size_t)b * T + t) * d + c];
  if ((rc = upload_f16(m, vt.data(), vt.size(), &dvt))) return rc;
  if ((rc = dev_alloc_t(&dout, n))) return rc;
  fwk::launch_attn_enc(m->stream, dq, dk, d, (int64_t)T * d, dvt, tp, (int64_t)d * tp, dout, d, (int64_t)T * d, B, H,
                       T);
  rc = download_f16(m, dout, n, out);
  for (half_t* p : {dq, dk, dvt, dout})
    if (p) (void)hipFree(p);
  return rc;
}

int32_t fw_bench_attention(fw_model* fm, int32_t B, int32_t H, int32_t T, int32_t variant, int32_t iters, float* ms_out) {
  FW_CHECK_ARG(fm && ms_out && B > 0 && H > 0 && T > 0 && iters > 0, "bad argument");
  Model* m = &fm->impl;
  std::lock_guard<std::mutex> lk(m->mu);
  FW_HIP(hipSetDevice(m->device));
  const int d = H * 64, tp = (T + 63) / 64 * 64;
  const size_t nqk = (size_t)B * T * 2 * d, nvt = (size_t)B * d * tp, no = (size_t)B * T * d;
  half_t *dqk = nullptr, *dvt = nullptr, *dout = nullptr;
  int rc;
  auto cleanup = [&]() { for (half_t* p : {dqk, dvt, dout}) if (p) (void)hipFree(p); };
  if ((rc = dev_alloc_t(&dqk, nqk)) || (rc = dev_alloc_t(&dvt, nvt)) || (rc = dev_alloc_t(&dout, no))) { cleanup(); return rc; }
  {
    std::vector<uint16_t> h(std::max(nqk, nvt));
    uint32_t sd = 777u;
    for (auto& v : h) { sd = sd * 1664525u + 1013904223u; v = f32_to_f16_bits(((int)(sd >> 16) % 2001 - 1000) * 2e-3f); }
    FW_HIP(hipMemcpy(dqk, h.data(), nqk * 2, hipMemcpyHostToDevice));
    FW_HIP(hipMemcpy(dvt, h.data(), nvt * 2, hipMemcpyHostToDevice));
  }
  hipEvent_t e0, e1;
  FW_HIP(hipEventCreate(&e0));
  FW_HIP(hipEventCreate(&e1));
  auto go = [&]() {
    fwk::launch_attn_enc(m->stream, dqk, dqk + d, 2 * d, (int64_t)T * 2 * d, dvt, tp, (int64_t)d * tp, dout, d, (int64_t)T * d, B,
                         H, T, variant);
  };
  go();
  FW_HIP(hipEventRecord(e0, m->stream));
  for (int i = 0; i < iters; ++i) go();
  FW_HIP(hipEventRecord(e1, m->stream));
  hipError_t he = hipEventSynchronize(e1);
  float ms = 0.f;
  if (he == hipSuccess) he = hipEventElapsedTime(&ms, e0, e1);
  (void)hipEventDestroy(e0);
  (void)hipEventDestroy(e1);
  cleanup();
  if (he != hipSuccess) { set_error("attention bench failed: %s", hipGetErrorString(he)); return FW_ERUNTIME; }
  *ms_out = ms / (float)iters;
  return FW_OK;
}

extern "C++" {
namespace {
struct DevBufs {
  std::vector<void*> p;
  template <typename T>
  int alloc(T** dst, size_t n) {
    int rc = dev_alloc_t(dst, n);
    if (!rc) p.push_back(*dst);
    return rc;
  }
  ~DevBufs() { for (void* q : p) (void)hipFree(q); }
};
int upload_f16_to(const float* src, size_t n, half_t* dst) {
  std::vector<uint16_t> tmp(n);
  for (size_t i = 0; i < n; ++i) tmp[i] = f32_to_f16_bits(src[i]);
  FW_HIP(hipMemcpy(dst, tmp.data(), n * 2, hipMemcpyHostToDevice));
  return FW_OK;
}
}
}

int32_t fw_test_dec_self_attn(fw_model* fm, const float* qkv, float* kcache, float* vcache, const uint8_t* kvidx,
                              int32_t n_chunks, int32_t kmul, int32_t Kbeam, int32_t H, int32_t n_ctx, int32_t cache_ctx,
                              int32_t pos_fixed, int32_t P, int32_t step, int32_t blk_n, int32_t frag, float* out) {
  FW_CHECK_ARG(fm && qkv && kcache && vcache && kvidx && out, "null argument");
  FW_CHECK_ARG(n_chunks >= 1 && H >= 1 && kmul >= 1 && kmul <= 16 && Kbeam >= 1 && Kbeam <= 255, "bad geometry");
  FW_CHECK_ARG(n_ctx >= 1 && n_ctx <= 448 && cache_ctx >= 1 && cache_ctx <= n_ctx, "need 1 <= cache_ctx <= n_ctx <= 448");
  FW_CHECK_ARG(blk_n >= 0 && (blk_n == 0 ? kmul <= Kbeam : (kmul == blk_n && pos_fixed >= 0)),
               "blk_n = 0: kmul <= Kbeam; blk_n > 0: kmul == blk_n and pos_fixed >= 0");
  const int pos0 = pos_fixed >= 0 ? pos_fixed : P - 1 + step;
  const int pos_last = pos0 + (blk_n > 0 ? blk_n - 1 : 0);
  FW_CHECK_ARG(pos0 >= 0 && pos_last < cache_ctx, "positions %d..%d outside the cache (%d)", pos0, pos_last, cache_ctx);
  const int d = H * 64, R = n_chunks * kmul, R16 = (R + 15) / 16 * 16, R_total = n_chunks * Kbeam;
  FW_CHECK_ARG(blk_n == 0 || fwd::self_attn_block_ok(n_ctx, cache_ctx, d, R_total), "position blocks need n_ctx %% 4 == 0");
  const size_t n_tab = (size_t)2 * R_total * n_ctx, n_cache = (size_t)R_total * H * cache_ctx * 64;
  for (size_t i = 0; i < n_tab; ++i)
    FW_CHECK_ARG(kvidx[i] < Kbeam, "kvidx[%zu] = %d is not a beam of %d", i, (int)kvidx[i], Kbeam);
  Model* m = &fm->impl;
  std::lock_guard<std::mutex> lk(m->mu);
  FW_HIP(hipSetDevice(m->device));
  DevBufs db;
  half_t *d_qkv, *d_kc, *d_vc, *d_out;
  uint8_t* d_idx;
  int* d_step;
  int rc;
  if ((rc = db.alloc(&d_qkv, (size_t)R * 3 * d)) || (rc = db.alloc(&d_kc, n_cache)) || (rc = db.alloc(&d_vc, n_cache)) ||
      (rc = db.alloc(&d_out, (size_t)R16 * d)) || (rc = db.alloc(&d_idx, n_tab)) || (rc = db.alloc(&d_step, 1)))
    return rc;
  if ((rc = upload_f16_to(qkv, (size_t)R * 3 * d, d_qkv)) || (rc = upload_f16_to(kcache, n_cache, d_kc)) ||
      (rc = upload_f16_to(vcache, n_cache, d_vc)))
    return rc;
  FW_HIP(hipMemcpy(d_idx, kvidx, n_tab, hipMemcpyHostToDevice));
  FW_HIP(hipMemcpy(d_step, &step, sizeof(int), hipMemcpyHostToDevice));
  FW_HIP(hipMemset(d_out, 0, (size_t)R16 * d * 2));
  fwd::launch_self_attn(m->stream, d_qkv, d, d_kc, d_vc, n_ctx, cache_ctx, H, d_idx, Kbeam, kmul, d_out, R, d_step,
                        pos_fixed, P, R_total, frag ? 1 : 0, blk_n);
  FW_HIP(hipGetLastError());
  if ((rc = download_f16(m, d_kc, n_cache, kcache)) || (rc = download_f16(m, d_vc, n_cache, vcache))) return rc;
  if (!frag) return download_f16(m, d_out, (size_t)R * d, out);
  std::vector<float> of((size_t)R16 * d);
  if ((rc = download_f16(m, d_out, of.size(), of.data()))) return rc;
  for (int r = 0; r < R; ++r)
    for (int n = 0; n < d; ++n) out[(size_t)r * d + n] = of[frag_pos(r, n, d, 32)];
  return FW_OK;
}

int32_t fw_test_dec_cross_attn(fw_model* fm, const float* q, const float* k, const float* v, int32_t n_enc, int32_t T,
                               int32_t H, int32_t B, int32_t kmul, int32_t kv_div, const int32_t* slot_map,
                               const int32_t* done, int32_t frag, float k_pad, float* out) {
  FW_CHECK_ARG(fm && q && k && v && slot_map && out, "null argument");
  FW_CHECK_ARG(n_enc >= 1 && T >= 1 && H >= 1 && B >= 1 && kmul >= 1 && kmul <= 16 && kv_div >= 1, "bad geometry");
  const int n_map = (B + kv_div - 1) / kv_div;
  for (int i = 0; i < n_map; ++i)
    FW_CHECK_ARG(slot_map[i] >= 0 && slot_map[i] < n_enc, "slot_map[%d] = %d outside [0, %d)", i, slot_map[i], n_enc);
  const int d = H * 64, kvp = (T + 31) / 32 * 32, R = B * kmul, R16 = (R + 15) / 16 * 16;
  const size_t blk = (size_t)d * kvp;
  std::vector<float> kf((size_t)n_enc * blk), vf((size_t)n_enc * blk, 0.f);
  for (int e = 0; e < n_enc; ++e)
    for (int t = 0; t < kvp; ++t)
      for (int n = 0; n < d; ++n) {
        const size_t src = ((size_t)e * T + t) * d + n;
        kf[e * blk + cross_kv_frag_pos(false, kvp, t, n)] = t < T ? k[src] : k_pad;
        if (t < T) vf[e * blk + cross_kv_frag_pos(true, kvp, t, n)] = v[src];
      }
  std::vector<float> of((size_t)R16 * d, 0.f);
  if (frag)
    for (int r = 0; r < R; ++r)
      for (int n = 0; n < d; ++n) of[frag_pos(r, n, d, 32)] = out[(size_t)r * d + n];
  Model* m = &fm->impl;
  std::lock_guard<std::mutex> lk(m->mu);
  FW_HIP(hipSetDevice(m->device));
  DevBufs db;
  half_t *d_q, *d_k, *d_vt, *d_out;
  int *d_map, *d_done = nullptr;
  int rc;
  if ((rc = db.alloc(&d_q, (size_t)R * d)) || (rc = db.alloc(&d_k, kf.size())) || (rc = db.alloc(&d_vt, vf.size())) ||
      (rc = db.alloc(&d_out, (size_t)R16 * d)) || (rc = db.alloc(&d_map, (size_t)n_map)) || (done && (rc = db.alloc(&d_done, (size_t)B))))
    return rc;
  if ((rc = upload_f16_to(q, (size_t)R * d, d_q)) || (rc = upload_f16_to(kf.data(), kf.size(), d_k)) ||
      (rc = upload_f16_to(vf.data(), vf.size(), d_vt)) || (rc = upload_f16_to(frag ? of.data() : out, frag ? of.size() : (size_t)R * d, d_out)))
    return rc;
  FW_HIP(hipMemcpy(d_map, slot_map, (size_t)n_map * sizeof(int), hipMemcpyHostToDevice));
  if (done) FW_HIP(hipMemcpy(d_done, done, (size_t)B * sizeof(int), hipMemcpyHostToDevice));
  fwd::launch_cross_attn(m->stream, d_q, d, d_k, d_vt, T, kvp, kmul, d_out, B, H, d_done, kv_div, frag ? 1 : 0, d_map);
  FW_HIP(hipGetLastError());
  if (!frag) return download_f16(m, d_out, (size_t)R * d, out);
  if ((rc = download_f16(m, d_out, of.size(), of.data()))) return rc;
  for (int r = 0; r < R; ++r)
    for (int n = 0; n < d; ++n) out[(size_t)r * d + n] = of[frag_pos(r, n, d, 32)];
  return FW_OK;
}

int32_t fw_test_dec_cross_probs(fw_model* fm, const float* q, const float* k, int32_t B, int32_t T, int32_t H,
                                const int32_t* heads, int32_t n_sel, int32_t n_tok, int32_t tok_idx, int32_t blk_n,
                                float* probs) {
  FW_CHECK_ARG(fm && q && k && heads && probs, "null argument");
  const int blk = blk_n > 0 ? blk_n : 1;
  FW_CHECK_ARG(B >= 1 && T >= 1 && H >= 1 && n_sel >= 1 && blk_n >= 0 && blk <= 16, "bad geometry");
  FW_CHECK_ARG(tok_idx >= 0 && tok_idx + blk <= n_tok, "tokens %d..%d outside [0, %d)", tok_idx, tok_idx + blk - 1, n_tok);
  for (int i = 0; i < n_sel; ++i) FW_CHECK_ARG(heads[i] >= 0 && heads[i] < H, "heads[%d] = %d outside [0, %d)", i, heads[i], H);
  const int d = H * 64, kvp = (T + 31) / 32 * 32;
  const size_t blkk = (size_t)d * kvp, n_probs = (size_t)B * n_sel * n_tok * T;
  std::vector<float> kf((size_t)B * blkk, 0.f);
  for (int b = 0; b < B; ++b)
    for (int t = 0; t < T; ++t)
      for (int n = 0; n < d; ++n) kf[b * blkk + cross_kv_frag_pos(false, kvp, t, n)] = k[((size_t)b * T + t) * d + n];
  Model* m = &fm->impl;
  std::lock_guard<std::mutex> lk(m->mu);
  FW_HIP(hipSetDevice(m->device));
  DevBufs db;
  half_t *d_q, *d_k;
  int* d_heads;
  float* d_p;
  int rc;
  if ((rc = db.alloc(&d_q, (size_t)B * blk * d)) || (rc = db.alloc(&d_k, kf.size())) || (rc = db.alloc(&d_heads, (size_t)n_sel)) ||
      (rc = db.alloc(&d_p, n_probs)))
    return rc;
  if ((rc = upload_f16_to(q, (size_t)B * blk * d, d_q)) || (rc = upload_f16_to(kf.data(), kf.size(), d_k))) return rc;
  FW_HIP(hipMemcpy(d_heads, heads, (size_t)n_sel * sizeof(int), hipMemcpyHostToDevice));
  FW_HIP(hipMemcpy(d_p, probs, n_probs * sizeof(float), hipMemcpyHostToDevice));
  fwd::launch_cross_probs(m->stream, d_q, d, d_k, T, kvp, d_heads, n_sel, n_sel, d_p, n_tok, tok_idx, B, blk_n);
  FW_HIP(hipGetLastError());
  FW_HIP(hipStreamSynchronize(m->stream));
  FW_HIP(hipMemcpy(probs, d_p, n_probs * sizeof(float), hipMemcpyDeviceToHost));
  return FW_OK;
}

int32_t fw_test_dec_softmax_pick(fw_model* fm, const float* logits, int32_t rows, int32_t V, int32_t row_mul,
                                 const int32_t* target, int32_t nospeech, float* out) {
  FW_CHECK_ARG(fm && logits && target && out, "null argument");
  FW_CHECK_ARG(rows >= 1 && V >= 1 && row_mul >= 1, "bad geometry");
  FW_CHECK_ARG(!nospeech || (target[0] >= 0 && target[0] < V), "no-speech id %d outside [0, %d)", target[0], V);
  Model* m = &fm->impl;
  std::lock_guard<std::mutex> lk(m->mu);
  FW_HIP(hipSetDevice(m->device));
  DevBufs db;
  const size_t n_lg = (size_t)rows * row_mul * V;
  float *d_lg, *d_out;
  int* d_t;
  int rc;
  if ((rc = db.alloc(&d_lg, n_lg)) || (rc = db.alloc(&d_out, (size_t)rows)) || (rc = db.alloc(&d_t, (size_t)rows))) return rc;
  FW_HIP(hipMemcpy(d_lg, logits, n_lg * sizeof(float), hipMemcpyHostToDevice));
  FW_HIP(hipMemcpy(d_t, target, (size_t)(nospeech ? 1 : rows) * sizeof(int), hipMemcpyHostToDevice));
  if (nospeech) fwd::launch_nospeech(m->stream, d_lg, V, row_mul, target[0], d_out, rows);
  else fwd::launch_token_prob(m->stream, d_lg, V, d_t, d_out, 1, 0, rows, row_mul);
  FW_HIP(hipGetLastError());
  FW_HIP(hipStreamSynchronize(m->stream));
  FW_HIP(hipMemcpy(out, d_out, (size_t)rows * sizeof(float), hipMemcpyDeviceToHost));
  return FW_OK;
}

}
```

faster_whisper_amd/csrc/gemm.hip:

```cpp
#include "common.h"
#include "kernels.h"
#include <atomic>
#include <type_traits>

#define GB_M 256
#define GB_N 256
#define GB_UNIT_BYTES (128 * 128)
#define GB_SLOT_BYTES (4 * GB_UNIT_BYTES)
#define GB_LDS_BYTES (8 * 64 * 272)

typedef int intx16 __attribute__((ext_vector_type(16)));

#ifndef GB_TL
#define GB_TL(slot)
#endif

#define GB_BARRIER()                      \
  do {                                    \
    asm volatile("" ::: "memory");         \
    __builtin_amdgcn_s_barrier();         \
    asm volatile("" ::: "memory");         \
  } while (0)

template <bool TRANS, bool I8, bool LAYERED = false>
__global__ __launch_bounds__(512) void gemm_f16_kernel(fwk::GemmParams p) {
  extern __shared__ __attribute__((aligned(16))) char smem_raw[];
  constexpr int ES = I8 ? 1 : 2;

  const int tid = threadIdx.x;
  const int lane = tid & 63;
  const int wave = __builtin_amdgcn_readfirstlane(tid >> 6);
  const int hi = lane >> 5, l31 = lane & 31;
  const int wm = wave >> 2, wn = wave & 3;

  int bid = xcd_remap(blockIdx.x, gridDim.x);
  int mp, nt;
  if (p.blk_n > 0) {
    const int per_band = p.blk_m * p.nNt;
    const int band = bid / per_band, r = bid - band * per_band;
    int bm = p.n_mp - band * p.blk_m; if (bm > p.blk_m) bm = p.blk_m;
    const int per_blk = bm * p.blk_n;
    const int cb = r / per_blk, rr = r - cb * per_blk;
    const int mi = rr / p.blk_n;
    mp = band * p.blk_m + mi;
    nt = cb * p.blk_n + (rr - mi * p.blk_n);
  } else {
    mp = bid / p.nNt;
    nt = bid - mp * p.nNt;
  }
  const int z = mp / p.nMt;
  const int mt = mp - z * p.nMt;
  int layer = 0;
  if (LAYERED) { layer = nt / p.nNt_layer; nt -= layer * p.nNt_layer; }
  const int m0 = mt * GB_M, n0 = nt * GB_N;

  const char* Ab = reinterpret_cast<const char*>(p.A) + (size_t)z * p.a_bstride * ES;
  const char* Wb = reinterpret_cast<const char*>(p.W) + (LAYERED ? (size_t)layer * p.w_lstride * ES : 0);
  const half_t* const biasp = (LAYERED && p.bias) ? p.bias + (size_t)layer * p.bias_lstride : p.bias;
  half_t* const Cp = LAYERED ? p.C + (size_t)layer * p.c_lstride : p.C;

  unsigned goff[4][2];
#pragma unroll
  for (int i = 0; i < 2; ++i) {
    const int u = (i * 8 + wave) * 8 + (lane >> 3);
    const int c = (lane & 7) ^ ((u >> 1) & 7);
#pragma unroll
    for (int h = 0; h < 2; ++h) {
      int am = m0 + (u >> 6) * 128 + (u & 63) + h * 64; if (am > p.M - 1) am = p.M - 1;
      int wr = n0 + (u >> 5) * 64 + (u & 31) + h * 32; if (wr > p.N - 1) wr = p.N - 1;
      goff[h][i] = (unsigned)((size_t)am * p.lda * ES + c * 16);
      goff[2 + h][i] = (unsigned)((size_t)wr * p.ldw * ES + c * 16);
    }
  }
  const int nk = p.K * ES / 128;
  auto issue = [&](int unit, int kt) {
    char* dst = smem_raw + (kt & 1) * GB_SLOT_BYTES + unit * GB_UNIT_BYTES;
    const char* base = unit < 2 ? Ab : Wb;
    const unsigned koff = (unsigned)kt * 128u;
#pragma unroll
    for (int i = 0; i < 2; ++i)
      __builtin_amdgcn_global_load_lds((const __attribute__((address_space(1))) void*)(base + (size_t)(goff[unit][i] + koff)),
                                       (__attribute__((address_space(3))) void*)(dst + (i * 8 + wave) * 1024), 16, 0, 0);
  };

  floatx16 accf[4][2];
  intx16 acci[4][2];
#pragma unroll
  for (int i = 0; i < 4; ++i)
#pragma unroll
    for (int j = 0; j < 2; ++j) { accf[i][j] = floatx16{0}; acci[i][j] = intx16{0}; }

  int arow[2], akey[2];
#pragma unroll
  for (int i = 0; i < 2; ++i) {
    const int u = wm * 64 + i * 32 + l31;
    arow[i] = u * 128;
    akey[i] = (u >> 1) & 7;
  }
  const int bu = wn * 32 + l31;
  const int brow = bu * 128, bkey = (bu >> 1) & 7;

  intx4 fa[2][4], fb0[4], fb1[4];
  auto read_a = [&](const char* unit) {
#pragma unroll
    for (int i = 0; i < 2; ++i)
#pragma unroll
      for (int ks = 0; ks < 4; ++ks)
        fa[i][ks] = *reinterpret_cast<const intx4*>(unit + arow[i] + (((ks * 2 + hi) ^ akey[i]) << 4));
  };
  auto read_b = [&](const char* unit, intx4 (&fb)[4]) {
#pragma unroll
    for (int ks = 0; ks < 4; ++ks) fb[ks] = *reinterpret_cast<const intx4*>(unit + brow + (((ks * 2 + hi) ^ bkey) << 4));
  };
  auto mma = [&](int ah, int ni, const intx4 (&fb)[4]) {
    __builtin_amdgcn_s_setprio(1);
#pragma unroll
    for (int ks = 0; ks < 4; ++ks)
#pragma unroll
      for (int i = 0; i < 2; ++i) {
        const int mi = ah * 2 + i;
        const intx4 opa = TRANS ? fa[i][ks] : fb[ks];
        const intx4 opb = TRANS ? fb[ks] : fa[i][ks];
        if (I8) acci[mi][ni] = __builtin_amdgcn_mfma_i32_32x32x32_i8(opa, opb, acci[mi][ni], 0, 0, 0);
        else accf[mi][ni] = __builtin_amdgcn_mfma_f32_32x32x16_f16(__builtin_bit_cast(half8_t, opa),
                                                                 __builtin_bit_cast(half8_t, opb), accf[mi][ni], 0, 0, 0);
      }
    __builtin_amdgcn_s_setprio(0);
  };
  auto seg_wait = [&](bool issued) {
    if (issued) asm volatile("s_waitcnt vmcnt(8)" ::: "memory");
    else asm volatile("s_waitcnt vmcnt(0)" ::: "memory");
  };

  issue(2, 0); issue(0, 0); issue(3, 0); issue(1, 0);
  if (nk > 1) { issue(2, 1); issue(0, 1); }
  seg_wait(nk > 1);
  GB_BARRIER();
  if (wm == 1) GB_BARRIER();

  auto tile = [&](int kt, auto N1, auto N2) {
    constexpr bool n1 = decltype(N1)::value, n2 = decltype(N2)::value;
    const char* slot = smem_raw + (kt & 1) * GB_SLOT_BYTES;
    GB_TL(0);
    read_a(slot);
    read_b(slot + 2 * GB_UNIT_BYTES, fb0);
    if (n1) issue(3, kt + 1);
    seg_wait(n1);
    GB_TL(1);
    GB_BARRIER();
    GB_TL(2);
    mma(0, 0, fb0);
    GB_TL(3);
    GB_BARRIER();
    GB_TL(4);
    read_b(slot + 3 * GB_UNIT_BYTES, fb1);
    if (n1) issue(1, kt + 1);
    seg_wait(n1);
    GB_TL(5);
    GB_BARRIER();
    GB_TL(6);
    mma(0, 1, fb1);
    GB_TL(7);
    GB_BARRIER();
    GB_TL(8);
    read_a(slot + GB_UNIT_BYTES);
    if (n2) issue(2, kt + 2);
    seg_wait(n2);
    GB_TL(9);
    GB_BARRIER();
    GB_TL(10);
    mma(1, 0, fb0);
    GB_TL(11);
    GB_BARRIER();
    GB_TL(12);
    if (n2) issue(0, kt + 2);
    seg_wait(n2);
    GB_TL(13);
    GB_BARRIER();
    GB_TL(14);
    mma(1, 1, fb1);
    GB_TL(15);
    GB_BARRIER();
  };
  using T_ = std::true_type;
  using F_ = std::false_type;
  int kt = 0;
  for (; kt + 2 < nk; ++kt) tile(kt, T_{}, T_{});
  if (kt + 1 < nk) { tile(kt, T_{}, F_{}); ++kt; }
  if (kt < nk) tile(kt, F_{}, F_{});
  if (wm == 0) GB_BARRIER();

  const float* sa = I8 ? p.a_scale + (size_t)z * p.as_bstride : nullptr;
  if (!TRANS && p.head_rows == 0) {
    constexpr int EP_STRIDE = 272;
    char* ep = smem_raw + wave * (64 * EP_STRIDE);
    half_t* Cb = Cp + (size_t)z * p.c_bstride;
    const half_t* Rb = p.res ? p.res + (size_t)z * p.r_bstride : nullptr;
    const int mw = m0 + wm * 128, nw = n0 + wn * 64;
    const int rr = lane >> 3, cc = (lane & 7) * 8;
    const bool vec_ok = (p.ldc % 8 == 0) && (p.c_bstride % 8 == 0) && (!Rb || ((p.ldr % 8 == 0) && (p.r_bstride % 8 == 0)));
#pragma unroll
    for (int half = 0; half < 2; ++half) {
#pragma unroll
      for (int ni = 0; ni < 2; ++ni)
#pragma unroll
        for (int mh = 0; mh < 2; ++mh) {
          const int mi = half * 2 + mh;
          const int r = mh * 32 + l31;
          int mc = mw + half * 64 + r; if (mc > p.M - 1) mc = p.M - 1;
          const float sam = I8 ? sa[mc] : 1.f;
#pragma unroll
          for (int g = 0; g < 4; ++g) {
            const int c = ni * 32 + 8 * g + 4 * hi;
            int n = nw + c; if (n > p.N - 4) n = p.N - 4;
            floatx4 v;
#pragma unroll
            for (int e = 0; e < 4; ++e)
              v[e] = I8 ? (float)acci[mi][ni][g * 4 + e] * sam * p.w_scale[n + e] : accf[mi][ni][g * 4 + e];
            if (biasp) {
              const half4_t bv = *reinterpret_cast<const half4_t*>(biasp + n);
#pragma unroll
              for (int e = 0; e < 4; ++e) v[e] += (float)bv[e];
            }
            if (p.act == 1) {
#pragma unroll
              for (int e = 0; e < 4; ++e) v[e] = gelu_erf(v[e]);
            }
            *reinterpret_cast<floatx4*>(ep + r * EP_STRIDE + c * 4) = v;
          }
        }
#pragma unroll 4
      for (int j = 0; j < 8; ++j) {
        const int r = j * 8 + rr;
        const int m = mw + half * 64 + r, n = nw + cc;
        const floatx4 v0 = *reinterpret_cast<const floatx4*>(ep + r * EP_STRIDE + cc * 4);
        const floatx4 v1 = *reinterpret_cast<const floatx4*>(ep + r * EP_STRIDE + cc * 4 + 16);
        if (m >= p.M || n >= p.N) continue;
        float v[8] = {v0[0], v0[1], v0[2], v0[3], v1[0], v1[1], v1[2], v1[3]};
        if (vec_ok && n + 8 <= p.N) {
          if (Rb) {
            const half8_t rv = *reinterpret_cast<const half8_t*>(Rb + (size_t)m * p.ldr + n);
#pragma unroll
            for (int e = 0; e < 8; ++e) v[e] += (float)rv[e];
          }
          half8_t o;
#pragma unroll
          for (int e = 0; e < 8; ++e) o[e] = (half_t)v[e];
          *reinterpret_cast<half8_t*>(Cb + (size_t)m * p.ldc + n) = o;
        } else {
          for (int e = 0; e < 8 && n + e < p.N; ++e) {
            float t = v[e];
            if (Rb) t += (float)Rb[(size_t)m * p.ldr + n + e];
            Cb[(size_t)m * p.ldc + n + e] = (half_t)t;
          }
        }
      }
    }
  } else if (p.head_rows > 0) {
    constexpr int FS = 144;
    char* ep = smem_raw + wave * (64 * FS);
    half_t* Cb = Cp + (size_t)z * p.c_bstride;
    const int mw = m0 + wm * 128, nw = n0 + wn * 64;
    if (nw < p.N) {
      half_t* Hb = Cb + (size_t)(nw >> 6) * p.head_rows * 64;
      const int g4 = lane >> 4, j = lane & 15;
#pragma unroll
      for (int half = 0; half < 2; ++half) {
#pragma unroll
        for (int ni = 0; ni < 2; ++ni)
#pragma unroll
          for (int mh = 0; mh < 2; ++mh) {
            const int mi = half * 2 + mh;
            if (!TRANS) {
              const int r = mh * 32 + l31;
              int mc = mw + half * 64 + r; if (mc > p.M - 1) mc = p.M - 1;
              const float sam = I8 ? sa[mc] : 1.f;
#pragma unroll
              for (int g = 0; g < 4; ++g) {
                const int c = ni * 32 + 8 * g + 4 * hi;
                int n = nw + c; if (n > p.N - 4) n = p.N - 4;
                half4_t o;
#pragma unroll
                for (int e = 0; e < 4; ++e) {
                  float v = I8 ? (float)acci[mi][ni][g * 4 + e] * sam * p.w_scale[n + e] : accf[mi][ni][g * 4 + e];
                  if (biasp) v += (float)biasp[n + e];
                  if (p.act == 1) v = gelu_erf(v);
                  o[e] = (half_t)v;
                }
                *reinterpret_cast<half4_t*>(ep + r * FS + c * 2) = o;
              }
            } else {
              const int c = ni * 32 + l31;
              int n = nw + c; if (n > p.N - 1) n = p.N - 1;
              const float bv = biasp ? (float)biasp[n] : 0.f;
              const float swn = I8 ? p.w_scale[n] : 1.f;
#pragma unroll
              for (int g = 0; g < 4; ++g) {
                const int r = mh * 32 + 8 * g + 4 * hi;
                half4_t o;
#pragma unroll
                for (int e = 0; e < 4; ++e) {
                  int mm = mw + half * 64 + r + e; if (mm > p.M - 1) mm = p.M - 1;
                  float v = (I8 ? (float)acci[mi][ni][g * 4 + e] * swn * sa[mm] : accf[mi][ni][g * 4 + e]) + bv;
                  if (p.act == 1) v = gelu_erf(v);
                  o[e] = (half_t)v;
                }
                *reinterpret_cast<half4_t*>(ep + c * FS + r * 2) = o;
              }
            }
          }
#pragma unroll
        for (int gl = 0; gl < 2; ++gl) {
          const int key0 = mw + half * 64 + gl * 32;
          if (key0 >= p.M) continue;
          half_t* Gb = Hb + (size_t)(key0 >> 5) * 4 * 512;
#pragma unroll
          for (int q = 0; q < 4; ++q) {
            intx4 v;
            if (!TRANS) {
              const int kl = gl * 32 + 8 * (j >> 2) + 4 * (q >> 1) + (j & 3);
              v = *reinterpret_cast<const intx4*>(ep + kl * FS + (32 * (q & 1) + 8 * g4) * 2);
              if (mw + half * 64 + kl < p.M) *reinterpret_cast<intx4*>(Gb + ((size_t)q * 64 + lane) * 8) = v;
            } else {
              const int kl = gl * 32 + 8 * g4;
              v = *reinterpret_cast<const intx4*>(ep + (16 * q + j) * FS + kl * 2);
              const int left = p.M - (mw + half * 64 + kl);
              if (left <= 0) continue;
              if (left < 8) {
                half8_t h = __builtin_bit_cast(half8_t, v);
#pragma unroll
                for (int e = 0; e < 8; ++e)
                  if (e >= left) h[e] = (half_t)0.f;
                v = __builtin_bit_cast(intx4, h);
              }
              *reinterpret_cast<intx4*>(Gb + ((size_t)q * 64 + lane) * 8) = v;
            }
          }
        }
      }
    }
  } else if (TRANS && !I8 && p.vt_stage) {
    constexpr int TS = 272;
    char* ep = smem_raw + wave * (64 * TS);
    half_t* Cb = Cp + (size_t)z * p.c_bstride;
    const int mw = m0 + wm * 128, nw = n0 + wn * 64;
#pragma unroll
    for (int ni = 0; ni < 2; ++ni) {
      const int c = ni * 32 + l31;
      int n = nw + c; if (n > p.N - 1) n = p.N - 1;
      const float bv = biasp ? (float)biasp[n] : 0.f;
#pragma unroll
      for (int mi = 0; mi < 4; ++mi)
#pragma unroll
        for (int g = 0; g < 4; ++g) {
          const int r = mi * 32 + 8 * g + 4 * hi;
          half4_t o;
#pragma unroll
          for (int e = 0; e < 4; ++e) {
            float v = accf[mi][ni][g * 4 + e] + bv;
            if (p.act == 1) v = gelu_erf(v);
            o[e] = (half_t)v;
          }
          *reinterpret_cast<half4_t*>(ep + c * TS + r * 2) = o;
        }
    }
    const int rr = lane >> 4, cc = (lane & 15) * 8;
#pragma unroll 4
    for (int j = 0; j < 16; ++j) {
      const int c = j * 4 + rr;
      const int n = nw + c, m = mw + cc;
      const intx4 v = *reinterpret_cast<const intx4*>(ep + c * TS + cc * 2);
      if (n >= p.N || m >= p.M) continue;
      half_t* dst = Cb + (size_t)n * p.ldc + m;
      if (m + 8 <= p.M) {
        *reinterpret_cast<intx4*>(dst) = v;
      } else {
        const half8_t h = __builtin_bit_cast(half8_t, v);
#pragma unroll
        for (int e = 0; e < 8; ++e)
          if (m + e < p.M) dst[e] = h[e];
      }
    }
  } else {
    half_t* Cb = Cp + (size_t)z * p.c_bstride;
#pragma unroll
    for (int mi = 0; mi < 4; ++mi)
#pragma unroll
      for (int ni = 0; ni < 2; ++ni) {
        const int n = n0 + wn * 64 + ni * 32 + l31;
        if (n >= p.N) continue;
        const float bv = biasp ? (float)biasp[n] : 0.f;
        const float swn = I8 ? p.w_scale[n] : 1.f;
#pragma unroll
        for (int g = 0; g < 4; ++g) {
          const int m = m0 + wm * 128 + mi * 32 + 8 * g + 4 * hi;
          half4_t o;
#pragma unroll
          for (int e = 0; e < 4; ++e) {
            int mm = m + e; if (mm > p.M - 1) mm = p.M - 1;
            float v = (I8 ? (float)acci[mi][ni][g * 4 + e] * swn * sa[mm] : accf[mi][ni][g * 4 + e]) + bv;
            if (p.act == 1) v = gelu_erf(v);
            o[e] = (half_t)v;
          }
          half_t* dst = Cb + (size_t)n * p.ldc + m;
          if (m + 3 < p.M) {
            *reinterpret_cast<half4_t*>(dst) = o;
          } else {
#pragma unroll
            for (int e = 0; e < 4; ++e)
              if (m + e < p.M) dst[e] = o[e];
          }
        }
      }
  }
}

namespace fwk {

std::atomic<int> g_gemm_order{1};
std::atomic<int> g_gemm_vt_stage{1};

int launch_gemm(hipStream_t st, const GemmParams& pin, int batch, bool trans) {
  GemmParams p = pin;
  const bool i8 = p.a_scale != nullptr;
  const int es = i8 ? 1 : 2;
  if (p.K <= 0 || (p.K * es) % 128 != 0) return -1;
  if (((p.lda * es) % 16) || ((p.ldw * es) % 16) || ((p.a_bstride * es) % 16)) return -1;
  if (!trans && ((p.N % 4) || (p.ldc % 4) || (p.c_bstride % 4))) return -1;
  if (i8 && !p.w_scale) return -1;
  p.nMt = (p.M + GB_M - 1) / GB_M;
  p.nNt_layer = (p.N + GB_N - 1) / GB_N;
  if (p.n_layers > 1 && (i8 || p.res)) return -1;
  p.nNt = p.nNt_layer * (p.n_layers > 1 ? p.n_layers : 1);
  p.n_mp = p.nMt * batch;
  p.blk_m = p.blk_n = 0;
  p.vt_stage = (trans && !i8 && p.head_rows == 0 && g_gemm_vt_stage.load(std::memory_order_relaxed) == 1 && p.ldc % 8 == 0 &&
                p.c_bstride % 8 == 0) ? 1 : 0;
  if (g_gemm_order.load(std::memory_order_relaxed) == 1 && p.nNt > 1 && p.n_mp > 1) {
    int bn = 1, best = 1 << 30;
    for (int c = 1; c <= p.nNt && c <= 16; ++c) {
      if (p.nNt % c) continue;
      const int cost = c + (32 + c - 1) / c;
      if (cost <= best) { best = cost; bn = c; }
    }
    p.blk_n = bn;
    p.blk_m = 32 / bn > 1 ? 32 / bn : 1;
  }
  const int lds = GB_LDS_BYTES;
  static std::atomic<unsigned long long> attr_done{0};
  int dev = 0;
  (void)hipGetDevice(&dev);
  if (!((attr_done.load(std::memory_order_acquire) >> (dev & 63)) & 1ull)) {
    (void)hipFuncSetAttribute(reinterpret_cast<const void*>(gemm_f16_kernel<false, false>),
                              hipFuncAttributeMaxDynamicSharedMemorySize, lds);
    (void)hipFuncSetAttribute(reinterpret_cast<const void*>(gemm_f16_kernel<true, false>),
                              hipFuncAttributeMaxDynamicSharedMemorySize, lds);
    (void)hipFuncSetAttribute(reinterpret_cast<const void*>(gemm_f16_kernel<false, true>),
                              hipFuncAttributeMaxDynamicSharedMemorySize, lds);
    (void)hipFuncSetAttribute(reinterpret_cast<const void*>(gemm_f16_kernel<true, true>),
                              hipFuncAttributeMaxDynamicSharedMemorySize, lds);
    attr_done.fetch_or(1ull << (dev & 63), std::memory_order_release);
  }
  const int grid = p.nMt * p.nNt * batch;
  if (p.n_layers > 1) {
    static std::atomic<unsigned long long> attr_l{0};
    if (!((attr_l.load(std::memory_order_acquire) >> (dev & 63)) & 1ull)) {
      (void)hipFuncSetAttribute(reinterpret_cast<const void*>(gemm_f16_kernel<false, false, true>),
                                hipFuncAttributeMaxDynamicSharedMemorySize, lds);
      (void)hipFuncSetAttribute(reinterpret_cast<const void*>(gemm_f16_kernel<true, false, true>),
                                hipFuncAttributeMaxDynamicSharedMemorySize, lds);
      attr_l.fetch_or(1ull << (dev & 63), std::memory_order_release);
    }
    if (trans) gemm_f16_kernel<true, false, true><<<grid, 512, lds, st>>>(p);
    else gemm_f16_kernel<false, false, true><<<grid, 512, lds, st>>>(p);
    return 0;
  }
  if (i8) {
    if (trans) gemm_f16_kernel<true, true><<<grid, 512, lds, st>>>(p);
    else gemm_f16_kernel<false, true><<<grid, 512, lds, st>>>(p);
  } else {
    if (trans) gemm_f16_kernel<true, false><<<grid, 512, lds, st>>>(p);
    else gemm_f16_kernel<false, false><<<grid, 512, lds, st>>>(p);
  }
  return 0;
}

}
```

profiles/dec_linear_bench.py:

```python
import ctypes as C
import os
import sys

sys.path.insert(0, os.path.dirname(os.path.dirname(os.path.abspath(__file__))))
from faster_whisper_amd import Whisper, _lib, get_config, synthetic_weights

VARIANTS = {0: "4w 2x2 ch5 (product K<2560)", 1: "8w 2x2 ch5 (product K>=2560)", 2: "8w 4x2 ch3", 3: "8w 4x2 ch4",
            4: "8w 4x4 ch2", 5: "8w 4x4 ch3", 6: "4w 4x2 ch3", 7: "8w 2x4 ch3", 8: "8w 8x2 ch2", 9: "4w 4x4 ch2",
            10: "big 4x2 waves 256x128 KC2x3", 11: "big 2x2 waves 128x64 KC1x5", 12: "big 2x2 waves 128x128 KC1x4",
            13: "sp 4 slices x 2x2 waves 128x64 x3",
            21: "4w 4x4 ch5", 22: "8w 4x4 ch5", 23: "4w 1x1 ch10", 24: "8w 1x1 ch10", 25: "4w 1x2 ch6", 26: "8w 1x2 ch6"}
if os.environ.get("DLB_VARIANTS"):
    VARIANTS = {int(v): VARIANTS[int(v)] for v in os.environ["DLB_VARIANTS"].split(",")}
SHAPES = [("qkv", 3840, 1280, 1), ("dxd", 1280, 1280, 0), ("ffn1", 5120, 1280, 1), ("ffn2", 1280, 5120, 0)]
if os.environ.get("DLB_LNF") is not None:
    SHAPES = [(n, N, K, int(os.environ["DLB_LNF"])) for n, N, K, _ in SHAPES]


def main():
    cfg = get_config("micro")
    m = Whisper("synthetic:micro", device="cuda", files={"config": cfg, "weights": synthetic_weights(cfg, seed=1)},
                max_batch_size=1, max_beam_size=1)
    h = m._replicas[0].handle
    us = C.c_float()
    rows = [int(a) for a in sys.argv[1:]] or [80, 320, 640]
    for R in rows:
        print(f"R = {R}")
        print("  %-38s" % "variant" + "".join("%10s" % s[0] for s in SHAPES) + "   layer (qkv + 3 dxd + ffn1 + ffn2)   TFLOP/s")
        for v, name in VARIANTS.items():
            t = []
            for _, N, K, lnf in SHAPES:
                rc = m._lib.fw_bench_dec_linear(h, R, N, K, lnf, v, 400, C.byref(us))
                t.append(us.value if rc == 0 else float("nan"))
            layer = t[0] + 3 * t[1] + t[2] + t[3]
            flop = 2.0 * R * sum(n * k * (3 if nm == "dxd" else 1) for nm, n, k, _ in SHAPES)
            print("  %-38s" % name + "".join("%10.2f" % x for x in t) + "   %8.1f   %8.0f" % (layer, flop / layer / 1e6), flush=True)


if __name__ == "__main__":
    main()
```

profiles/gemm_bench.py:

```python
import argparse
import ctypes as C
import json
import os
import sys

sys.path.insert(0, os.path.dirname(os.path.dirname(os.path.abspath(__file__))))

SHAPES = [
    ("conv1", 3000, 1280, 384, 0), ("conv2", 1500, 1280, 3840, 0), ("qk", 1500, 2560, 1280, 0),
    ("v^T", 1500, 1280, 1280, 1), ("out", 1500, 1280, 1280, 0), ("ffn1", 1500, 5120, 1280, 0),
    ("ffn2", 1500, 1280, 5120, 0),
]


def main():
    ap = argparse.ArgumentParser()
    ap.add_argument("--int8", action="store_true")
    ap.add_argument("--pad", default="0")
    ap.add_argument("--batch", type=int, default=16)
    ap.add_argument("--iters", type=int, default=10)
    ap.add_argument("--order", type=int, default=-1, help="tile order of every launch (1 blocked, 0 n fastest); default: A/B")
    ap.add_argument("--square", default="",
                    help="comma-separated sizes n: time the kernel at n x n x n (batch 1) — the guide quotes its 256^2 "
                         "8-phase template at 4096^3 / 8192^3 on random operands (cdna_hip_programming.md), where a launch "
                         "is exactly one or four full rounds of 256 workgroups and K is 64-128 tiles deep; the encoder "
                         "shapes are 1.9-7.5 rounds and 6-80 K tiles")
    args = ap.parse_args()
    from faster_whisper_amd import Whisper, _lib, get_config, synthetic_weights
    cfg = get_config("micro")
    model = Whisper("synthetic:micro", device="cuda", files={"config": cfg, "weights": synthetic_weights(cfg, 3)},
                    compute_type="int8_float16" if args.int8 else "float16", max_batch_size=1, max_beam_size=1)
    lib = _lib.load()
    h = model._replicas[0].handle
    out = {"env": {k: v for k, v in os.environ.items() if k.startswith("FWAMD_")}, "int8": args.int8}
    if args.square:
        for n in [int(x) for x in args.square.split(",")]:
            ms = C.c_float()
            _lib.check(lib.fw_bench_gemm(h, n, n, n, 1, 0, 0, 0, args.iters, C.byref(ms)))
            out[f"square {n}"] = {"ms": round(ms.value, 4), "TFLOP/s": round(2.0 * n * n * n / ms.value / 1e9, 1)}
        print(json.dumps(out, indent=1))
        return
    weights = {"conv1": 1, "conv2": 1, "qk": 32, "v^T": 32, "out": 32, "ffn1": 32, "ffn2": 32}
    for pad in [int(x) for x in args.pad.split(",")]:
        tot = {1: [0.0, 0.0], 0: [0.0, 0.0]}
        for name, M, N, K, tr in SHAPES:
            for order in ((1, 0, 1, 0) if args.order < 0 else (args.order,)):
                _lib.check(lib.fw_test_knob(1, order))
                ms = C.c_float()
                _lib.check(lib.fw_bench_gemm(h, M, N, K, args.batch, pad, pad, tr, args.iters, C.byref(ms)))
                fl = 2.0 * args.batch * M * N * K
                key = f"{name} pad={pad} order={order}"
                prev = out.get(key)
                if prev is None or ms.value < prev["ms"]:
                    out[key] = {"ms": round(ms.value, 4), "TFLOP/s": round(fl / ms.value / 1e9, 1)}
            for order in ((1, 0) if args.order < 0 else (args.order,)):
                tot[order][0] += out[f"{name} pad={pad} order={order}"]["ms"] * weights[name]
                tot[order][1] += 2.0 * args.batch * M * N * K * weights[name]
        for order in ((1, 0) if args.order < 0 else (args.order,)):
            out[f"encoder-weighted pad={pad} order={order}"] = {"ms": round(tot[order][0], 2),
                                                               "TFLOP/s": round(tot[order][1] / tot[order][0] / 1e9, 1)}
    _lib.check(lib.fw_test_knob(1, 1))
    print(json.dumps(out, indent=1))


if __name__ == "__main__":
    main()
```

Measured before the change: 3094.

## Prefetch epilogue bias, LN constants and residuals before the K loop in GEMMs

Moves the per-column epilogue constants (bias, LayerNorm scale/shift, int8 weight scales) and the residual tiles out of the epilogue in the decoder frag/big/skinny kernels and the encoder GEMM. They are now loaded before or during the main K loop, with clamped indices instead of guarded loads, so their latency overlaps the MMA work instead of stalling the store path. It also adds an early exit for idle column groups in the skinny kernel, plus new epilogue benchmark entry points and scripts. The cost is higher register pressure from holding those values across the main loop, which is why some configurations defer the loads.

```diff
diff --git a/faster_whisper_amd/_lib.py b/faster_whisper_amd/_lib.py
--- a/faster_whisper_amd/_lib.py
+++ b/faster_whisper_amd/_lib.py
@@ -74,6 +74,7 @@
     "fw_dev_alloc", "fw_dev_free", "fw_dev_upload",
     "fw_test_gemm", "fw_test_layernorm", "fw_test_attention", "fw_test_dec_linear", "fw_test_dec_logits", "fw_test_logits_rules",
     "fw_test_dec_self_attn", "fw_test_dec_cross_attn", "fw_test_dec_cross_probs", "fw_test_dec_softmax_pick", "fw_bench_gemm", "fw_bench_dec_linear", "fw_bench_attention",
+    "fw_bench_gemm_epi", "fw_bench_dec_linear_epi",
     "fw_vad_create", "fw_vad_forward", "fw_vad_free", "fw_vad_forward_dev", "fw_vad_forward_audio_dev",
     "fw_flac_info", "fw_flac_decode",
 ]
@@ -167,6 +168,9 @@
     lib.fw_bench_attention.argtypes = [vp, i32, i32, i32, i32, i32, f32p]
     lib.fw_bench_gemm.argtypes = [vp, i32, i32, i32, i32, i32, i32, i32, i32, f32p]
     lib.fw_bench_dec_linear.argtypes = [vp, i32, i32, i32, i32, i32, i32, f32p]
+    if hasattr(lib, "fw_bench_gemm_epi"):
+        lib.fw_bench_gemm_epi.argtypes = [vp, i32, i32, i32, i32, i32, i32, i32, i32, i32, i32, i32, f32p]
+        lib.fw_bench_dec_linear_epi.argtypes = [vp, i32, i32, i32, i32, i32, i32, i32, i32, i32, f32p]
     lib.fw_test_layernorm.argtypes = [vp, vp, vp, vp, i32, i32, vp]
     lib.fw_test_attention.argtypes = [vp, vp, vp, vp, i32, i32, i32, vp]
     lib.fw_vad_create.argtypes = [C.POINTER(FwVadWeights), C.POINTER(vp)]
diff --git a/faster_whisper_amd/csrc/dec_kernels.hip b/faster_whisper_amd/csrc/dec_kernels.hip
--- a/faster_whisper_amd/csrc/dec_kernels.hip
+++ b/faster_whisper_amd/csrc/dec_kernels.hip
@@ -41,19 +41,26 @@
   const float var = ex2 - mu * mu;
   rstd = rsqrtf(fmaxf(var, 0.f) + 1e-5f);
 }
+struct DecColConsts { floatx4 a4, c4; half4_t b4; };
 template <bool LNF>
-static __device__ __forceinline__ half4_t dec_epilogue4(const floatx4 v, float mu, float rstd,
-                                                        const float* __restrict__ s1, const float* __restrict__ cf,
-                                                        const half_t* __restrict__ bias, bool has_res, half4_t r4, int n, int act) {
+static __device__ __forceinline__ DecColConsts dec_col_consts(const float* __restrict__ s1, const float* __restrict__ cf,
+                                                              const half_t* __restrict__ bias, int n) {
+  DecColConsts k;
+  k.a4 = floatx4{0.f, 0.f, 0.f, 0.f}; k.c4 = k.a4;
+  k.b4 = half4_t{(half_t)0.f, (half_t)0.f, (half_t)0.f, (half_t)0.f};
+  if (LNF) {
+    k.a4 = *reinterpret_cast<const floatx4*>(s1 + n);
+    k.c4 = *reinterpret_cast<const floatx4*>(cf + n);
+  } else if (bias) {
+    k.b4 = *reinterpret_cast<const half4_t*>(bias + n);
+  }
+  return k;
+}
+template <bool LNF>
+static __device__ __forceinline__ half4_t dec_epilogue4(const floatx4 v, float mu, float rstd, const floatx4 a4,
+                                                        const floatx4 c4, const half4_t b4, bool bias, bool has_res,
+                                                        half4_t r4, int act) {
 #pragma clang fp contract(off)
-  floatx4 a4 = {0.f, 0.f, 0.f, 0.f}, c4 = {0.f, 0.f, 0.f, 0.f};
-  half4_t b4 = {(half_t)0.f, (half_t)0.f, (half_t)0.f, (half_t)0.f};
-  if (LNF) {
-    a4 = *reinterpret_cast<const floatx4*>(s1 + n);
-    c4 = *reinterpret_cast<const floatx4*>(cf + n);
-  } else if (bias) {
-    b4 = *reinterpret_cast<const half4_t*>(bias + n);
-  }
   half4_t o;
 #pragma unroll
   for (int e = 0; e < 4; ++e) {
@@ -123,18 +130,24 @@
 #pragma unroll
     for (int b = 0; b < NT; ++b) acc[a][b] = floatx4{0, 0, 0, 0};
   }
+  constexpr bool CONSTS_EARLY = !(LNF && RT * NT > 1);
   half4_t resv[(RT * NT + WAVES - 1) / WAVES];
-#pragma unroll
-  for (int q = 0; q < (RT * NT + WAVES - 1) / WAVES; ++q) resv[q] = half4_t{(half_t)0.f, (half_t)0.f, (half_t)0.f, (half_t)0.f};
-  if (res) {
-#pragma unroll
-    for (int a = 0; a < RT; ++a) {
-#pragma unroll
-      for (int b = 0; b < NT; ++b) {
-        if ((a * NT + b) % WAVES != wave) continue;
-        const int row = (rt0 + a) * 16 + i, n = (ct0 + b) * 16 + 4 * g;
-        if (row < R && n < N) resv[(a * NT + b) / WAVES] = *reinterpret_cast<const half4_t*>(res + (size_t)row * ldr + n);
-      }
+  DecColConsts colk[(RT * NT + WAVES - 1) / WAVES];
+#pragma unroll
+  for (int q = 0; q < (RT * NT + WAVES - 1) / WAVES; ++q) {
+    resv[q] = half4_t{(half_t)0.f, (half_t)0.f, (half_t)0.f, (half_t)0.f};
+    colk[q] = DecColConsts{floatx4{0.f, 0.f, 0.f, 0.f}, floatx4{0.f, 0.f, 0.f, 0.f}, resv[q]};
+  }
+#pragma unroll
+  for (int a = 0; a < RT; ++a) {
+#pragma unroll
+    for (int b = 0; b < NT; ++b) {
+      if ((a * NT + b) % WAVES != wave) continue;
+      int row = (rt0 + a) * 16 + i, n = (ct0 + b) * 16 + 4 * g;
+      if (row > R - 1) row = R - 1;
+      if (n > N - 4) n = N - 4;
+      if (CONSTS_EARLY) colk[(a * NT + b) / WAVES] = dec_col_consts<LNF>(s1, cf, bias, n);
+      if (res) resv[(a * NT + b) / WAVES] = *reinterpret_cast<const half4_t*>(res + (size_t)row * ldr + n);
     }
   }
   if (nks > 0) {
@@ -184,6 +197,18 @@
       }
     }
   }
+  if (!CONSTS_EARLY) {
+#pragma unroll
+    for (int a = 0; a < RT; ++a) {
+#pragma unroll
+      for (int b = 0; b < NT; ++b) {
+        if ((a * NT + b) % WAVES != wave) continue;
+        int n = (ct0 + b) * 16 + 4 * g;
+        if (n > N - 4) n = N - 4;
+        colk[(a * NT + b) / WAVES] = dec_col_consts<LNF>(s1, cf, bias, n);
+      }
+    }
+  }
 #pragma unroll
   for (int a = 0; a < RT; ++a) {
     if (LNF) {
@@ -221,7 +246,8 @@
       if (n >= N) continue;
       const floatx4 v4 = {v[0], v[1], v[2], v[3]};
       const half4_t r4 = resv[(a * NT + b) / WAVES];
-      const half4_t o = dec_epilogue4<LNF>(v4, mu, rstd, s1, cf, bias, res != nullptr, r4, n, act);
+      const DecColConsts& ck = colk[(a * NT + b) / WAVES];
+      const half4_t o = dec_epilogue4<LNF>(v4, mu, rstd, ck.a4, ck.c4, ck.b4, bias != nullptr, res != nullptr, r4, act);
       if (out) *reinterpret_cast<half4_t*>(out + (size_t)row * ldo + n) = o;
       if (out_frag) *reinterpret_cast<half4_t*>(out_frag + frag_off(row, n, N >> 5)) = o;
     }
@@ -396,6 +422,33 @@
     slot = (slot + 1 == NST) ? 0 : slot + 1;
   }
   wait_vmcnt<0>();
+  const int row0 = (rt0 + wm * 4) * 16;
+  const int col0 = (ct0 + wn * FB) * 16;
+  constexpr int CPR = FB * 2;
+  constexpr int RPI = 64 / CPR;
+  const int cr = lane / CPR, cc = lane % CPR;
+  constexpr int NSEG = 64 / RPI;
+  constexpr int RES_EARLY = (LNF && NW == 8 && FB == 4) ? 2 : NSEG;
+  DecColConsts colk[FB];
+  intx4 resv[NSEG];
+  auto load_res = [&](int j0, int j1) {
+    if (!res) return;
+#pragma unroll
+    for (int j = 0; j < NSEG; ++j) {
+      if (j < j0 || j >= j1) continue;
+      int row = row0 + j * RPI + cr, n = col0 + cc * 8;
+      if (row > R - 1) row = R - 1;
+      if (n > N - 8) n = N - 8;
+      resv[j] = *reinterpret_cast<const intx4*>(res + (size_t)row * ldr + n);
+    }
+  };
+#pragma unroll
+  for (int b = 0; b < FB; ++b) {
+    int n = col0 + b * 16 + 4 * g;
+    if (n > N - 4) n = N - 4;
+    colk[b] = dec_col_consts<LNF>(s1, cf, bias, n);
+  }
+  load_res(0, RES_EARLY);
 #pragma unroll 1
   for (int c = n_steady; c < nch; ++c) {
     DGB_BARRIER();
@@ -403,6 +456,7 @@
     if (--to_slice == 0) { to_slice = ch_per_slice; slice_end(); }
     slot = (slot + 1 == NST) ? 0 : slot + 1;
   }
+  load_res(RES_EARLY, NSEG);
   DGB_BARRIER();
 
   if (LNF) {
@@ -424,19 +478,11 @@
     DGB_BARRIER_LDS();
   }
   char* ep = dgb_smem + wave * (64 * DGB_EP_STRIDE);
-  const int row0 = (rt0 + wm * 4) * 16;
-  const int col0 = (ct0 + wn * FB) * 16;
-  constexpr int CPR = FB * 2;
-  constexpr int RPI = 64 / CPR;
-  const int cr = lane / CPR, cc = lane % CPR;
   if (res) {
 #pragma unroll
     for (int j = 0; j < 64 / RPI; ++j) {
       const int r = j * RPI + cr;
-      const int row = row0 + r, n = col0 + cc * 8;
-      intx4 v = {0, 0, 0, 0};
-      if (row < R && n < N) v = *reinterpret_cast<const intx4*>(res + (size_t)row * ldr + n);
-      *reinterpret_cast<intx4*>(ep + r * DGB_EP_STRIDE + cc * 16) = v;
+      *reinterpret_cast<intx4*>(ep + r * DGB_EP_STRIDE + cc * 16) = resv[j];
     }
   }
 #pragma unroll
@@ -445,12 +491,11 @@
     if (LNF) dec_ln_stats(sa[a], sb[a], K, mu, rstd);
 #pragma unroll
     for (int b = 0; b < FB; ++b) {
-      int n = col0 + b * 16 + 4 * g;
-      if (n > N - 4) n = N - 4;
       char* cell = ep + (a * 16 + i) * DGB_EP_STRIDE + (b * 16 + 4 * g) * 2;
       half4_t r4 = {(half_t)0.f, (half_t)0.f, (half_t)0.f, (half_t)0.f};
       if (res) r4 = *reinterpret_cast<const half4_t*>(cell);
-      const half4_t o = dec_epilogue4<LNF>(tot[a][b], mu, rstd, s1, cf, bias, res != nullptr, r4, n, act);
+      const half4_t o = dec_epilogue4<LNF>(tot[a][b], mu, rstd, colk[b].a4, colk[b].c4, colk[b].b4, bias != nullptr,
+                                           res != nullptr, r4, act);
       *reinterpret_cast<half4_t*>(cell) = o;
     }
   }
@@ -579,6 +624,7 @@
   __shared__ float xst[SPLIT ? RT : 1][16][2];
   if (rt0 >= n_rt) return;
   if (!SPLIT && ct0 >= n_ct) return;
+  if (cgrp * WN * NT >= n_ct) return;
   const int KS = K / (I8 ? 64 : 32);
   const intx4* wp[NT];
   const intx4* xp[RT];
@@ -659,6 +705,20 @@
       }
     }
   };
+  float ks1[NT][4], kcf[NT][4], kws[NT][4];
+  half_t kb[NT][4];
+#pragma unroll
+  for (int b = 0; b < NT; ++b) {
+#pragma unroll
+    for (int e = 0; e < 4; ++e) {
+      const int n = (ct0 + b) * 16 + 4 * g + e;
+      const int ne = n < N ? n : N - 1;
+      ks1[b][e] = kcf[b][e] = 0.f; kws[b][e] = 1.f; kb[b][e] = (half_t)0.f;
+      if (I8) kws[b][e] = w_scale[ne];
+      if (LNF) { ks1[b][e] = s1[ne]; kcf[b][e] = cf[ne]; }
+      else if (bias) kb[b][e] = bias[ne];
+    }
+  }
   Set fa, fb;
   load(fa, 0);
   for (int ks0 = 0; ks0 < KS; ks0 += 2 * CH) {
@@ -704,10 +764,9 @@
       float t4[4];
 #pragma unroll
       for (int e = 0; e < 4; ++e) {
-        const int ne = n + e < N ? n + e : N - 1;
-        float tv = I8 ? (float)acci[a][b][e] * sx * w_scale[ne] : accf[a][b][e];
-        if (LNF) tv = rstd * (tv - mu * s1[ne]) + cf[ne];
-        else if (bias) tv += (float)bias[ne];
+        float tv = I8 ? (float)acci[a][b][e] * sx * kws[b][e] : accf[a][b][e];
+        if (LNF) tv = rstd * (tv - mu * ks1[b][e]) + kcf[b][e];
+        else if (bias) tv += (float)kb[b][e];
         t4[e] = tv;
       }
       if (F32 && pair_ok) {
diff --git a/faster_whisper_amd/csrc/engine.hip b/faster_whisper_amd/csrc/engine.hip
--- a/faster_whisper_amd/csrc/engine.hip
+++ b/faster_whisper_amd/csrc/engine.hip
@@ -1988,6 +1988,150 @@
   return FW_OK;
 }
 
+static int bench_fill(half_t* dst, size_t n, std::vector<uint16_t>& h, uint32_t seed) {
+  if (h.size() < n) h.resize(n);
+  for (size_t i = 0; i < n; ++i) { seed = seed * 1664525u + 1013904223u; h[i] = f32_to_f16_bits(((int)(seed >> 16) % 2001 - 1000) * 1e-3f); }
+  FW_HIP(hipMemcpy(dst, h.data(), n * 2, hipMemcpyHostToDevice));
+  return FW_OK;
+}
+
+int32_t fw_bench_gemm_epi(fw_model* fm, int32_t M, int32_t N, int32_t K, int32_t batch, int32_t lda_in, int32_t trans,
+                          int32_t bias, int32_t act, int32_t res, int32_t n_layers, int32_t iters, float* ms_out) {
+  FW_CHECK_ARG(fm && ms_out && M > 0 && N > 0 && K > 0 && batch > 0 && iters > 0 && n_layers >= 1, "bad argument");
+  FW_CHECK_ARG(res >= 0 && res <= 2 && !(res && (trans || n_layers > 1)), "residual: row-major single-layer output only");
+  Model* m = &fm->impl;
+  FW_CHECK_ARG(m->compute_type != FW_COMPUTE_INT8_FLOAT16, "float16 models only");
+  std::lock_guard<std::mutex> lk(m->mu);
+  FW_HIP(hipSetDevice(m->device));
+  const int64_t lda = lda_in > 0 ? lda_in : K;
+  const bool layered = n_layers > 1;
+  const int64_t kvp = (M + 31) / 32 * 32;
+  const int64_t ldct = layered ? kvp : (M + 63) / 64 * 64;
+  const int64_t c_bs = layered ? (int64_t)N * kvp : (trans ? (int64_t)N * ldct : (int64_t)M * N);
+  const int64_t c_ls = c_bs * batch;
+  const size_t na = (size_t)batch * ((size_t)M * lda + K), nw = (size_t)N * K * n_layers, nc = (size_t)c_ls * n_layers;
+  const size_t nr1 = res == 1 ? (size_t)batch * M * N : (size_t)M * N;
+  const int copies = res == 1 ? (int)std::max<size_t>(2, ((size_t)640 << 20) / (nr1 * 2)) : 1;
+  half_t *dA = nullptr, *dW = nullptr, *dC = nullptr, *dB = nullptr, *dR = nullptr;
+  int rc;
+  auto cleanup = [&]() { for (void* p : {(void*)dA, (void*)dW, (void*)dC, (void*)dB, (void*)dR}) if (p) (void)hipFree(p); };
+  if ((rc = dev_alloc_t(&dA, na)) || (rc = dev_alloc_t(&dW, nw)) || (rc = dev_alloc_t(&dC, nc)) ||
+      (rc = dev_alloc_t(&dB, (size_t)N * n_layers)) || (res && (rc = dev_alloc_t(&dR, nr1 * copies)))) {
+    cleanup();
+    return rc;
+  }
+  {
+    std::vector<uint16_t> h;
+    if ((rc = bench_fill(dA, na, h, 12345u)) || (rc = bench_fill(dW, nw, h, 12345u)) ||
+        (rc = bench_fill(dB, (size_t)N * n_layers, h, 777u))) { cleanup(); return rc; }
+    if (res) {
+      if ((rc = bench_fill(dR, nr1, h, 4242u))) { cleanup(); return rc; }
+      for (int c = 1; c < copies; ++c) FW_HIP(hipMemcpy(dR + (size_t)c * nr1, dR, nr1 * 2, hipMemcpyDeviceToDevice));
+    }
+    FW_HIP(hipMemset(dC, 0, nc * 2));
+  }
+  fwk::GemmParams p;
+  memset(&p, 0, sizeof(p));
+  p.A = dA; p.lda = lda; p.a_bstride = (int64_t)M * lda;
+  p.W = dW; p.ldw = K;
+  p.bias = bias ? dB : nullptr;
+  p.C = dC; p.ldc = layered ? (trans ? kvp : N) : (trans ? ldct : N); p.c_bstride = c_bs;
+  p.M = M; p.N = N; p.K = K;
+  p.act = act;
+  if (layered) {
+    p.head_rows = (int)kvp;
+    p.n_layers = n_layers; p.w_lstride = (int64_t)N * K; p.bias_lstride = N; p.c_lstride = c_ls;
+  }
+  p.ldr = N; p.r_bstride = res == 1 ? (int64_t)M * N : 0;
+  hipEvent_t e0, e1;
+  FW_HIP(hipEventCreate(&e0));
+  FW_HIP(hipEventCreate(&e1));
+  p.res = dR;
+  int lr = fwk::launch_gemm(m->stream, p, batch, trans != 0);
+  FW_HIP(hipEventRecord(e0, m->stream));
+  for (int i = 0; i < iters && lr == 0; ++i) {
+    if (res) p.res = dR + (size_t)(i % copies) * nr1;
+    lr = fwk::launch_gemm(m->stream, p, batch, trans != 0);
+  }
+  FW_HIP(hipEventRecord(e1, m->stream));
+  hipError_t he = hipEventSynchronize(e1);
+  float ms = 0.f;
+  if (he == hipSuccess) he = hipEventElapsedTime(&ms, e0, e1);
+  (void)hipEventDestroy(e0);
+  (void)hipEventDestroy(e1);
+  cleanup();
+  if (lr != 0 || he != hipSuccess) {
+    set_error("gemm epilogue bench failed: %s", lr ? "unsupported shape" : hipGetErrorString(he));
+    return FW_ERUNTIME;
+  }
+  *ms_out = ms / (float)iters;
+  return FW_OK;
+}
+
+int32_t fw_bench_dec_linear_epi(fw_model* fm, int32_t R, int32_t N, int32_t K, int32_t lnf, int32_t variant, int32_t act,
+                                int32_t res, int32_t outs, int32_t iters, float* us_out) {
+  FW_CHECK_ARG(fm && us_out && R > 0 && N > 0 && K > 0 && iters > 0, "bad argument");
+  FW_CHECK_ARG((outs & 3) != 0 && (!res || (outs & 1)), "needs an output; the residual is the row-major output in place");
+  FW_CHECK_ARG(variant == 0 || variant == 5 || (variant >= 10 && variant <= 12), "unknown variant %d", variant);
+  Model* m = &fm->impl;
+  std::lock_guard<std::mutex> lk(m->mu);
+  FW_HIP(hipSetDevice(m->device));
+  const size_t wn = (size_t)N * K;
+  const int copies = (int)std::max<size_t>(2, ((size_t)640 << 20) / (wn * 2));
+  const size_t rp = ((size_t)R + 15) / 16 * 16, on = rp * N;
+  const int ocopies = (int)std::max<size_t>(2, ((size_t)640 << 20) / (on * 2));
+  half_t *dW = nullptr, *dX = nullptr, *dO = nullptr, *dF = nullptr, *dB = nullptr;
+  float *dS = nullptr, *dC = nullptr;
+  int rc;
+  auto cleanup = [&]() { for (void* p : {(void*)dW, (void*)dX, (void*)dO, (void*)dF, (void*)dB, (void*)dS, (void*)dC}) if (p) (void)hipFree(p); };
+  if ((rc = dev_alloc_t(&dW, wn * copies)) || (rc = dev_alloc_t(&dX, rp * K)) || (rc = dev_alloc_t(&dO, on * ocopies)) ||
+      (rc = dev_alloc_t(&dF, on)) || (rc = dev_alloc_t(&dB, (size_t)N)) || (rc = dev_alloc_t(&dS, (size_t)N)) ||
+      (rc = dev_alloc_t(&dC, (size_t)N))) {
+    cleanup();
+    return rc;
+  }
+  {
+    std::vector<uint16_t> h;
+    if ((rc = bench_fill(dW, wn, h, 2463534242u)) || (rc = bench_fill(dX, rp * K, h, 2463534242u))) { cleanup(); return rc; }
+    for (int c = 1; c < copies; ++c) FW_HIP(hipMemcpy(dW + (size_t)c * wn, dW, wn * 2, hipMemcpyDeviceToDevice));
+  }
+  FW_HIP(hipMemset(dO, 0, on * ocopies * 2));
+  FW_HIP(hipMemset(dB, 0, (size_t)N * 2));
+  FW_HIP(hipMemset(dS, 0, (size_t)N * 4));
+  FW_HIP(hipMemset(dC, 0, (size_t)N * 4));
+  hipEvent_t e0, e1;
+  FW_HIP(hipEventCreate(&e0));
+  FW_HIP(hipEventCreate(&e1));
+  hipStream_t st = m->stream;
+  auto go = [&](int i) -> int {
+    const half_t* w = dW + (size_t)(i % copies) * wn;
+    half_t* o = dO + (size_t)(i % ocopies) * on;
+    half_t* op = (outs & 1) ? o : nullptr;
+    half_t* of = (outs & 2) ? dF : nullptr;
+    const half_t* r = res ? o : nullptr;
+    const half_t* b = lnf ? nullptr : dB;
+    const float *s1 = lnf ? dS : nullptr, *cf = lnf ? dC : nullptr;
+    if (variant >= 10) return fwd::launch_dec_gemm_big(st, variant - 10, dX, w, b, s1, cf, r, N, op, N, of, R, N, K, act);
+    if (variant == 5) return fwd::launch_dec_gemm_skinny(st, dX, w, b, s1, cf, r, N, op, N, of, R, N, K, act);
+    return fwd::launch_dec_gemm_frag(st, dX, w, b, s1, cf, r, N, op, N, of, R, N, K, act);
+  };
+  int lr = 0;
+  for (int i = 0; i < 4 && lr == 0; ++i) lr = go(i);
+  FW_HIP(hipEventRecord(e0, st));
+  for (int i = 0; i < iters && lr == 0; ++i) lr = go(i);
+  FW_HIP(hipEventRecord(e1, st));
+  hipError_t he = hipEventSynchronize(e1);
+  float ms = 0.f;
+  if (he == hipSuccess) he = hipEventElapsedTime(&ms, e0, e1);
+  (void)hipEventDestroy(e0);
+  (void)hipEventDestroy(e1);
+  cleanup();
+  if (lr != 0) { set_error("fw_bench_dec_linear_epi: unsupported shape / variant"); return FW_EINVAL; }
+  if (he != hipSuccess) { set_error("fw_bench_dec_linear_epi: %s", hipGetErrorString(he)); return FW_ENODEV; }
+  *us_out = ms * 1000.f / (float)iters;
+  return FW_OK;
+}
+
 int32_t fw_test_layernorm(fw_model* fm, const float* x, const float* g, const float* b, int32_t rows, int32_t d,
                           float* out) {
   FW_CHECK_ARG(fm && x && g && b && out, "null argument");
diff --git a/faster_whisper_amd/csrc/gemm.hip b/faster_whisper_amd/csrc/gemm.hip
--- a/faster_whisper_amd/csrc/gemm.hip
+++ b/faster_whisper_amd/csrc/gemm.hip
@@ -132,6 +132,41 @@
     else asm volatile("s_waitcnt vmcnt(0)" ::: "memory");
   };
 
+  const int mw = m0 + wm * 128, nw = n0 + wn * 64;
+  const bool rowmajor = !TRANS && p.head_rows == 0;
+  const half_t* const Rb = (rowmajor && p.res) ? p.res + (size_t)z * p.r_bstride : nullptr;
+  const int ep_rr = lane >> 3, ep_cc = (lane & 7) * 8;
+  const bool vec_ok = (p.ldc % 8 == 0) && (p.c_bstride % 8 == 0) && (!Rb || ((p.ldr % 8 == 0) && (p.r_bstride % 8 == 0)));
+  const half4_t hz4 = {(half_t)0.f, (half_t)0.f, (half_t)0.f, (half_t)0.f};
+  half4_t bias4[2][4] = {{hz4, hz4, hz4, hz4}, {hz4, hz4, hz4, hz4}};
+  half_t biasT[2] = {(half_t)0.f, (half_t)0.f};
+  half8_t resv[8];
+  auto load_bias = [&]() {
+    if (!biasp) return;
+#pragma unroll
+    for (int ni = 0; ni < 2; ++ni) {
+      if (TRANS) {
+        int n = nw + ni * 32 + l31; if (n > p.N - 1) n = p.N - 1;
+        biasT[ni] = biasp[n];
+      } else {
+#pragma unroll
+        for (int g = 0; g < 4; ++g) {
+          int n = nw + ni * 32 + 8 * g + 4 * hi; if (n > p.N - 4) n = p.N - 4;
+          bias4[ni][g] = *reinterpret_cast<const half4_t*>(biasp + n);
+        }
+      }
+    }
+  };
+  auto load_res = [&](int half) {
+    if (!Rb || !vec_ok || p.N < 8) return;
+#pragma unroll
+    for (int j = 0; j < 8; ++j) {
+      int m = mw + half * 64 + j * 8 + ep_rr; if (m > p.M - 1) m = p.M - 1;
+      int n = nw + ep_cc; if (n + 8 > p.N) n = (p.N - 8) & ~7;
+      resv[j] = *reinterpret_cast<const half8_t*>(Rb + (size_t)m * p.ldr + n);
+    }
+  };
+
   issue(2, 0); issue(0, 0); issue(3, 0); issue(1, 0);
   if (nk > 1) { issue(2, 1); issue(0, 1); }
   seg_wait(nk > 1);
@@ -175,6 +210,7 @@
     GB_TL(12);
     if (n2) issue(0, kt + 2);
     seg_wait(n2);
+    if (!n1 && !n2) { load_bias(); if (!I8) load_res(0); }
     GB_TL(13);
     GB_BARRIER();
     GB_TL(14);
@@ -195,12 +231,10 @@
     constexpr int EP_STRIDE = 272;
     char* ep = smem_raw + wave * (64 * EP_STRIDE);
     half_t* Cb = Cp + (size_t)z * p.c_bstride;
-    const half_t* Rb = p.res ? p.res + (size_t)z * p.r_bstride : nullptr;
-    const int mw = m0 + wm * 128, nw = n0 + wn * 64;
-    const int rr = lane >> 3, cc = (lane & 7) * 8;
-    const bool vec_ok = (p.ldc % 8 == 0) && (p.c_bstride % 8 == 0) && (!Rb || ((p.ldr % 8 == 0) && (p.r_bstride % 8 == 0)));
+    const int rr = ep_rr, cc = ep_cc;
 #pragma unroll
     for (int half = 0; half < 2; ++half) {
+      if (half == 1 || I8) load_res(half);
 #pragma unroll
       for (int ni = 0; ni < 2; ++ni)
 #pragma unroll
@@ -218,9 +252,8 @@
             for (int e = 0; e < 4; ++e)
               v[e] = I8 ? (float)acci[mi][ni][g * 4 + e] * sam * p.w_scale[n + e] : accf[mi][ni][g * 4 + e];
             if (biasp) {
-              const half4_t bv = *reinterpret_cast<const half4_t*>(biasp + n);
-#pragma unroll
-              for (int e = 0; e < 4; ++e) v[e] += (float)bv[e];
+#pragma unroll
+              for (int e = 0; e < 4; ++e) v[e] += (float)bias4[ni][g][e];
             }
             if (p.act == 1) {
 #pragma unroll
@@ -229,7 +262,7 @@
             *reinterpret_cast<floatx4*>(ep + r * EP_STRIDE + c * 4) = v;
           }
         }
-#pragma unroll 4
+#pragma unroll
       for (int j = 0; j < 8; ++j) {
         const int r = j * 8 + rr;
         const int m = mw + half * 64 + r, n = nw + cc;
@@ -239,7 +272,7 @@
         float v[8] = {v0[0], v0[1], v0[2], v0[3], v1[0], v1[1], v1[2], v1[3]};
         if (vec_ok && n + 8 <= p.N) {
           if (Rb) {
-            const half8_t rv = *reinterpret_cast<const half8_t*>(Rb + (size_t)m * p.ldr + n);
+            const half8_t rv = resv[j];
 #pragma unroll
             for (int e = 0; e < 8; ++e) v[e] += (float)rv[e];
           }
@@ -260,7 +293,6 @@
     constexpr int FS = 144;
     char* ep = smem_raw + wave * (64 * FS);
     half_t* Cb = Cp + (size_t)z * p.c_bstride;
-    const int mw = m0 + wm * 128, nw = n0 + wn * 64;
     if (nw < p.N) {
       half_t* Hb = Cb + (size_t)(nw >> 6) * p.head_rows * 64;
       const int g4 = lane >> 4, j = lane & 15;
@@ -283,7 +315,7 @@
 #pragma unroll
                 for (int e = 0; e < 4; ++e) {
                   float v = I8 ? (float)acci[mi][ni][g * 4 + e] * sam * p.w_scale[n + e] : accf[mi][ni][g * 4 + e];
-                  if (biasp) v += (float)biasp[n + e];
+                  if (biasp) v += (float)bias4[ni][g][e];
                   if (p.act == 1) v = gelu_erf(v);
                   o[e] = (half_t)v;
                 }
@@ -292,7 +324,7 @@
             } else {
               const int c = ni * 32 + l31;
               int n = nw + c; if (n > p.N - 1) n = p.N - 1;
-              const float bv = biasp ? (float)biasp[n] : 0.f;
+              const float bv = (float)biasT[ni];
               const float swn = I8 ? p.w_scale[n] : 1.f;
 #pragma unroll
               for (int g = 0; g < 4; ++g) {
@@ -343,12 +375,10 @@
     constexpr int TS = 272;
     char* ep = smem_raw + wave * (64 * TS);
     half_t* Cb = Cp + (size_t)z * p.c_bstride;
-    const int mw = m0 + wm * 128, nw = n0 + wn * 64;
 #pragma unroll
     for (int ni = 0; ni < 2; ++ni) {
       const int c = ni * 32 + l31;
-      int n = nw + c; if (n > p.N - 1) n = p.N - 1;
-      const float bv = biasp ? (float)biasp[n] : 0.f;
+      const float bv = (float)biasT[ni];
 #pragma unroll
       for (int mi = 0; mi < 4; ++mi)
 #pragma unroll
@@ -389,7 +419,7 @@
       for (int ni = 0; ni < 2; ++ni) {
         const int n = n0 + wn * 64 + ni * 32 + l31;
         if (n >= p.N) continue;
-        const float bv = biasp ? (float)biasp[n] : 0.f;
+        const float bv = (float)biasT[ni];
         const float swn = I8 ? p.w_scale[n] : 1.f;
 #pragma unroll
         for (int g = 0; g < 4; ++g) {
diff --git a/profiles/dec_linear_bench.py b/profiles/dec_linear_bench.py
--- a/profiles/dec_linear_bench.py
+++ b/profiles/dec_linear_bench.py
@@ -16,6 +16,27 @@
 if os.environ.get("DLB_LNF") is not None:
     SHAPES = [(n, N, K, int(os.environ["DLB_LNF"])) for n, N, K, _ in SHAPES]
 
+EPI_SHAPES = [("qkv", 3840, 1280, 1, 0, 0, 1), ("out", 1280, 1280, 0, 0, 1, 3), ("cross-q", 1280, 1280, 1, 0, 0, 1),
+              ("cross-out", 1280, 1280, 0, 0, 1, 3), ("ffn1", 5120, 1280, 1, 1, 0, 2), ("ffn2", 1280, 5120, 0, 0, 1, 3)]
+
+
+def epilogue_table(m, h, rows, reps=3, iters=400):
+    us = C.c_float()
+    for R in rows:
+        print(f"R = {R}   us per launch, min .. max of {reps} measurements (bare = no activation / residual, row-major output only)")
+        layer = {"bare": 0.0, "product": 0.0}
+        for name, N, K, lnf, act, res, outs in EPI_SHAPES:
+            t = {"bare": [], "product": []}
+            for _ in range(reps):
+                for key, (a_, r_, o_) in (("bare", (0, 0, 1)), ("product", (act, res, outs))):
+                    _lib.check(m._lib.fw_bench_dec_linear_epi(h, R, N, K, lnf, 0, a_, r_, o_, iters, C.byref(us)))
+                    t[key].append(us.value)
+            for key in t:
+                layer[key] += min(t[key])
+            print("  %-10s bare %7.2f .. %7.2f   product %7.2f .. %7.2f" %
+                  (name, min(t["bare"]), max(t["bare"]), min(t["product"]), max(t["product"])), flush=True)
+        print("  %-10s bare %7.2f              product %7.2f" % ("layer", layer["bare"], layer["product"]), flush=True)
+
 
 def main():
     cfg = get_config("micro")
@@ -23,6 +44,9 @@
                 max_batch_size=1, max_beam_size=1)
     h = m._replicas[0].handle
     us = C.c_float()
+    if "--epilogue" in sys.argv[1:]:
+        epilogue_table(m, h, [int(a) for a in sys.argv[1:] if a != "--epilogue"] or [80, 800, 1280])
+        return
     rows = [int(a) for a in sys.argv[1:]] or [80, 320, 640]
     for R in rows:
         print(f"R = {R}")
diff --git a/profiles/gemm_bench.py b/profiles/gemm_bench.py
--- a/profiles/gemm_bench.py
+++ b/profiles/gemm_bench.py
@@ -12,6 +12,35 @@
     ("ffn2", 1500, 1280, 5120, 0),
 ]
 
+EPI_SHAPES = [
+    ("conv1", 3000, 1280, 384, 128, 0, 1, 1, 0, 1), ("conv2", 1500, 1280, 3840, 2560, 0, 1, 1, 2, 1),
+    ("qk", 1500, 2560, 1280, 0, 0, 1, 0, 0, 1), ("v^T", 1500, 1280, 1280, 0, 1, 1, 0, 0, 1),
+    ("out", 1500, 1280, 1280, 0, 0, 1, 0, 1, 1), ("ffn1", 1500, 5120, 1280, 0, 0, 1, 1, 0, 1),
+    ("ffn2", 1500, 1280, 5120, 0, 0, 1, 0, 1, 1),
+    ("cross-K x32", 1500, 1280, 1280, 0, 0, 1, 0, 0, 32), ("cross-V^T x32", 1500, 1280, 1280, 0, 1, 1, 0, 0, 32),
+]
+
+
+def epilogue_table(lib, h, args):
+    from faster_whisper_amd import _lib
+    out = {"env": {k: v for k, v in os.environ.items() if k.startswith("FWAMD_")}}
+    for name, M, N, K, lda, tr, bias, act, res, layers in EPI_SHAPES:
+        fl = 2.0 * args.batch * M * N * K * layers
+        t = {"bare": [], "product": []}
+        for _ in range(args.reps):
+            for key, (b_, a_, r_) in (("bare", (0, 0, 0)), ("product", (bias, act, res))):
+                ms = C.c_float()
+                _lib.check(lib.fw_bench_gemm_epi(h, M, N, K, args.batch, lda, tr, b_, a_, r_, layers, args.iters, C.byref(ms)))
+                t[key].append(ms.value)
+        out[name] = {k: {"ms_min": round(min(v), 4), "ms_max": round(max(v), 4), "TFLOP/s": round(fl / min(v) / 1e9, 1)}
+                     for k, v in t.items()}
+    w = {"conv1": 1, "conv2": 1, "qk": 32, "v^T": 32, "out": 32, "ffn1": 32, "ffn2": 32}
+    for key in ("bare", "product"):
+        ms = sum(out[n][key]["ms_min"] * k for n, k in w.items())
+        fl = sum(2.0 * args.batch * M * N * K * w[n] for n, M, N, K, *_ in EPI_SHAPES if n in w)
+        out[f"encoder-weighted {key}"] = {"ms": round(ms, 2), "TFLOP/s": round(fl / ms / 1e9, 1)}
+    print(json.dumps(out, indent=1))
+
 
 def main():
     ap = argparse.ArgumentParser()
@@ -20,6 +49,8 @@
     ap.add_argument("--batch", type=int, default=16)
     ap.add_argument("--iters", type=int, default=10)
     ap.add_argument("--order", type=int, default=-1, help="tile order of every launch (1 blocked, 0 n fastest); default: A/B")
+    ap.add_argument("--epilogue", action="store_true", help="every shape with the epilogue the product runs for it")
+    ap.add_argument("--reps", type=int, default=3, help="--epilogue: measurements per shape and form")
     ap.add_argument("--square", default="",
                     help="comma-separated sizes n: time the kernel at n x n x n (batch 1) — the guide quotes its 256^2 "
                          "8-phase template at 4096^3 / 8192^3 on random operands (cdna_hip_programming.md), where a launch "
@@ -33,6 +64,9 @@
     lib = _lib.load()
     h = model._replicas[0].handle
     out = {"env": {k: v for k, v in os.environ.items() if k.startswith("FWAMD_")}, "int8": args.int8}
+    if args.epilogue:
+        epilogue_table(lib, h, args)
+        return
     if args.square:
         for n in [int(x) for x in args.square.split(",")]:
             ms = C.c_float()
```

New measurement: 3163 (median of 6 runs). 1.02x the previous value.
